# mahilab/mahi-mpc

Hardware: AMD Instinct MI355X
Metric: MPC solves/sec (whole node), nx=4 N=30 batch, at 1/2/4/8 MI355X (higher is better)
Workload: dtype f64; 1 GPU; cfg#2: 2-link arm nx=4 nu=2, N=30, h=2 ms, cold-start SQP (exact or Gauss-Newton Hessian: config.hessian) to ||grad||<=1e-8, ||g||<=1e-10; batch_per_gpu=4096, global_batch=4096, horizon=30, kkt_solver=riccati (16 lanes per instance), hessian=exact (Lagrangian, IPOPT's default), init_states=reference cold start V = 0 (MMPC_INIT_ZERO: V not read)

## Files before the change

### mahi-mpc_amd/csrc/fast_trig.h

```cpp
#pragma once
#include <math.h>

#ifndef MMPC_TRIG_FN
#if defined(__HIPCC__)
#define MMPC_TRIG_FN __device__ __forceinline__
#else
#define MMPC_TRIG_FN inline
#endif
#endif

namespace mmpc {

#define MMPC_TRIG_CONSTANTS                                                                                        \
    {0.63661977236758134308, 1.5707963267948966, 6.123233995736766e-17, -1.4973849048591698e-33,                 \
     -1.66666666666666324348e-01, 8.33333333332248946124e-03, -1.98412698298579493134e-04,                       \
     2.75573137070700676789e-06, -2.50507602534068634195e-08, 1.58969099521155010221e-10,                        \
     4.16666666666666019037e-02, -1.38888888888741095749e-03, 2.48015872894767294178e-05,                        \
     -2.75573143513906633035e-07, 2.08757232129817482790e-09, -1.13596475577881948265e-11}

#if defined(__HIPCC__)
__constant__ double kTrigConst[16] = MMPC_TRIG_CONSTANTS;
using trig_cptr = __attribute__((address_space(4))) const double*;
__device__ __forceinline__ trig_cptr trig_table() {
    trig_cptr K = (trig_cptr)kTrigConst;
    asm volatile("" : "+s"(K));
    return K;
}
#else
static const double kTrigConst[16] = MMPC_TRIG_CONSTANTS;
using trig_cptr = const double*;
inline trig_cptr trig_table() { return kTrigConst; }
#endif
#undef MMPC_TRIG_CONSTANTS

MMPC_TRIG_FN void sincos_fast(trig_cptr K, double x, double* s, double* c) {
#if !defined(__HIPCC__) && !defined(MMPC_TRIG_DEVICE_PATH_ON_HOST)
    if (!(fabs(x) <= 1647099.3291652855)) {
        *s = sin(x);
        *c = cos(x);
        return;
    }
#endif
    const double n = rint(x * K[0]);
    double r = fma(-n, K[1], x);
    r = fma(-n, K[2], r);
    r = fma(-n, K[3], r);
    r = fabs(x) <= 1647099.3291652855 ? r : __builtin_nan("");
    const double z = r * r;
    const double ps = fma(z, fma(z, fma(z, fma(z, K[9], K[8]), K[7]), K[6]), K[5]);
    const double sr = fma(z * r, fma(z, ps, K[4]), r);
    const double pc = z * fma(z, fma(z, fma(z, fma(z, fma(z, K[15], K[14]), K[13]), K[12]), K[11]), K[10]);
    const double hz = 0.5 * z;
    const double w = 1.0 - hz;
    const double cr = w + (((1.0 - w) - hz) + z * pc);
    const int q = (int)fma(-4.0, floor(0.25 * n), n);
    const bool odd = (q & 1) != 0;
    const double a = odd ? cr : sr, b = odd ? sr : cr;
    *s = (q & 2) ? -a : a;
    *c = ((q + 1) & 2) ? -b : b;
}

}
```

### mahi-mpc_amd/csrc/models.h

```cpp
#pragma once
#include <type_traits>

#include "device.h"
#include "exo_model_gen.h"
#include "two_link_fast.h"

namespace mmpc {

struct TwoLinkArm {
    static constexpr int NX = 4;
    static constexpr int NU = 2;
    static constexpr int NQ = 2;
    MMPC_HD static void eval(const double* x, const double* u, double* xd) { TwoLinkFast::eval(x, u, xd); }
    MMPC_HD static void eval_jac(const double* x, const double* u, double* xd, double* fx, double* fu) {
        double Fq[4], Fqd[4], Fu[4];
        TwoLinkFast::eval_acc_jac(x, u, xd + 2, Fq, Fqd, Fu);
        xd[0] = x[2];
        xd[1] = x[3];
#pragma unroll
        for (int r = 0; r < 2; ++r) {
#pragma unroll
            for (int c = 0; c < 4; ++c) fx[r * 4 + c] = (c == 2 + r) ? 1.0 : 0.0;
            fu[r * 2] = fu[r * 2 + 1] = 0.0;
#pragma unroll
            for (int c = 0; c < 2; ++c) {
                fx[(2 + r) * 4 + c] = Fq[r * 2 + c];
                fx[(2 + r) * 4 + 2 + c] = Fqd[r * 2 + c];
                fu[(2 + r) * 2 + c] = Fu[r * 2 + c];
            }
        }
    }
    MMPC_HD static void eval_acc_jac(const double* x, const double* u, double* acc, double* Fq, double* Fqd,
                                     double* Fu) {
        TwoLinkFast::eval_acc_jac(x, u, acc, Fq, Fqd, Fu);
    }
    static constexpr bool kHasHess = true;
    MMPC_HD static void eval_hess(const double* x, const double* u, const double* lam, double* W) {
        TwoLinkFast::eval_hess(x, u, lam, W);
    }
    static constexpr bool kControlAffine = true;
};

template <class M, class = void>
struct HasHess {
    static constexpr bool value = false;
};
template <class M>
struct HasHess<M, std::enable_if_t<M::kHasHess>> {
    static constexpr bool value = true;
};
template <class M, class = void>
struct IsControlAffine {
    static constexpr bool value = false;
};
template <class M>
struct IsControlAffine<M, std::enable_if_t<M::kControlAffine>> {
    static constexpr bool value = true;
};

template <class M, class = void>
struct HasJvp {
    static constexpr bool value = false;
};
template <class M>
struct HasJvp<M, std::enable_if_t<M::kHasJvp>> {
    static constexpr bool value = true;
};
template <class M, class = void>
struct HasJacH {
    static constexpr bool value = false;
};
template <class M>
struct HasJacH<M, std::enable_if_t<M::kHasJacH>> {
    static constexpr bool value = true;
};
template <class M>
MMPC_HD void model_acc_jac_h(const double* x, const double* u, double h, double* acc, double* hFq, double* hFqd,
                             double* hFu) {
    if constexpr (HasJacH<M>::value) M::eval_acc_jac_h(x, u, h, acc, hFq, hFqd, hFu);
}
template <class M>
MMPC_HD void model_jvp(const double* x, const double* u, const double* vx, const double* vu, double* xd, double* jv) {
    if constexpr (HasJvp<M>::value) M::eval_jvp(x, u, vx, vu, xd, jv);
}

struct ExoArm {
    static constexpr int NX = 8;
    static constexpr int NU = 4;
    static constexpr int NQ = 4;

    MMPC_HD static void chol4(const double* a, double* l, double* il) {
        sqrt_rsqrt(a[0], l[0], il[0]);
        l[1] = a[1] * il[0];
        l[3] = a[2] * il[0];
        l[6] = a[3] * il[0];
        sqrt_rsqrt(a[4] - l[1] * l[1], l[2], il[1]);
        l[4] = (a[5] - l[3] * l[1]) * il[1];
        l[7] = (a[6] - l[6] * l[1]) * il[1];
        sqrt_rsqrt(a[7] - l[3] * l[3] - l[4] * l[4], l[5], il[2]);
        l[8] = (a[8] - l[6] * l[3] - l[7] * l[4]) * il[2];
        sqrt_rsqrt(a[9] - l[6] * l[6] - l[7] * l[7] - l[8] * l[8], l[9], il[3]);
    }
    MMPC_HD static void chol4_solve(const double* l, const double* il, const double* b, double* y) {
        const double z0 = b[0] * il[0];
        const double z1 = (b[1] - l[1] * z0) * il[1];
        const double z2 = (b[2] - l[3] * z0 - l[4] * z1) * il[2];
        const double z3 = (b[3] - l[6] * z0 - l[7] * z1 - l[8] * z2) * il[3];
        y[3] = z3 * il[3];
        y[2] = (z2 - l[8] * y[3]) * il[2];
        y[1] = (z1 - l[4] * y[2] - l[7] * y[3]) * il[1];
        y[0] = (z0 - l[1] * y[1] - l[3] * y[2] - l[6] * y[3]) * il[0];
    }

    MMPC_HD static void eval(const double* x, const double* u, double* xd) {
        double s[4], c[4];
        const trig_cptr TK = trig_table();
#pragma unroll
        for (int i = 0; i < 4; ++i) sincos_fast(TK, x[i], &s[i], &c[i]);
        const exo::TrigPowers tp(c[1], c[2], c[3], s[1], s[2], s[3]);
        double Mu[10];
        exo::mass_upper(tp, Mu);
        double l[10], il[4], w[4];
#pragma unroll
        for (int i = 0; i < 4; ++i) w[i] = u[i] - exo::kDamping[i] * x[4 + i] - exo::kGravityGain[i] * s[i];
        chol4(Mu, l, il);
#pragma unroll
        for (int i = 0; i < 4; ++i) xd[i] = x[4 + i];
        chol4_solve(l, il, w, xd + 4);
    }

    template <int J>
    MMPC_HD static void dmass_times(const exo::TrigPowers& tp, const double* v, double* out) {
        double dM[10];
        exo::dmass_upper<J>(tp, dM);
        out[0] = fma(dM[0], v[0], fma(dM[1], v[1], fma(dM[2], v[2], dM[3] * v[3])));
        out[1] = fma(dM[1], v[0], fma(dM[4], v[1], fma(dM[5], v[2], dM[6] * v[3])));
        out[2] = fma(dM[2], v[0], fma(dM[5], v[1], fma(dM[7], v[2], dM[8] * v[3])));
        out[3] = fma(dM[3], v[0], fma(dM[6], v[1], fma(dM[8], v[2], dM[9] * v[3])));
    }

    MMPC_HD static void eval_acc_jac(const double* x, const double* u, double* qdd, double* Fq, double* Fqd,
                                     double* Fu) {
        double s[4], c[4];
        const trig_cptr TK = trig_table();
#pragma unroll
        for (int i = 0; i < 4; ++i) sincos_fast(TK, x[i], &s[i], &c[i]);
        const exo::TrigPowers tp(c[1], c[2], c[3], s[1], s[2], s[3]);
        double Mu[10], l[10], il[4], w[4];
        exo::mass_upper(tp, Mu);
#pragma unroll
        for (int i = 0; i < 4; ++i) w[i] = u[i] - exo::kDamping[i] * x[4 + i] - exo::kGravityGain[i] * s[i];
        chol4(Mu, l, il);
        chol4_solve(l, il, w, qdd);
#pragma unroll
        for (int j = 0; j < 4; ++j) {
            double e[4] = {0.0, 0.0, 0.0, 0.0}, col[4];
            e[j] = 1.0;
            chol4_solve(l, il, e, col);
#pragma unroll
            for (int r = 0; r < 4; ++r) Fu[r * 4 + j] = col[r];
        }
        double rhs[4][4];
#pragma unroll
        for (int r = 0; r < 4; ++r) rhs[0][r] = 0.0;
        dmass_times<1>(tp, qdd, rhs[1]);
        dmass_times<2>(tp, qdd, rhs[2]);
        dmass_times<3>(tp, qdd, rhs[3]);
#pragma unroll
        for (int j = 0; j < 4; ++j) {
#pragma unroll
            for (int r = 0; r < 4; ++r) rhs[j][r] = -rhs[j][r];
            rhs[j][j] -= exo::kGravityGain[j] * c[j];
#pragma unroll
            for (int r = 0; r < 4; ++r) {
                double t = 0.0;
#pragma unroll
                for (int cc = 0; cc < 4; ++cc) t = fma(Fu[r * 4 + cc], rhs[j][cc], t);
                Fq[r * 4 + j] = t;
                Fqd[r * 4 + j] = -Fu[r * 4 + j] * exo::kDamping[j];
            }
        }
    }

    static constexpr bool kHasJvp = true;
    MMPC_HD static void eval_jvp(const double* x, const double* u, const double* vx, const double* vu, double* xd,
                                 double* jv) {
        double s[4], c[4];
        const trig_cptr TK = trig_table();
#pragma unroll
        for (int i = 0; i < 4; ++i) sincos_fast(TK, x[i], &s[i], &c[i]);
        const exo::TrigPowers tp(c[1], c[2], c[3], s[1], s[2], s[3]);
        double Mu[10], l[10], il[4], w[4];
        exo::mass_upper(tp, Mu);
#pragma unroll
        for (int i = 0; i < 4; ++i) w[i] = u[i] - exo::kDamping[i] * x[4 + i] - exo::kGravityGain[i] * s[i];
        chol4(Mu, l, il);
#pragma unroll
        for (int i = 0; i < 4; ++i) xd[i] = x[4 + i];
        double* const qdd = xd + 4;
        chol4_solve(l, il, w, qdd);
        double r[4], t1[4], t2[4], t3[4];
        dmass_times<1>(tp, qdd, t1);
        dmass_times<2>(tp, qdd, t2);
        dmass_times<3>(tp, qdd, t3);
#pragma unroll
        for (int i = 0; i < 4; ++i) {
            double t = fma(-exo::kDamping[i], vx[4 + i], vu[i]);
            t = fma(-exo::kGravityGain[i] * c[i], vx[i], t);
            t = fma(-vx[1], t1[i], t);
            t = fma(-vx[2], t2[i], t);
            r[i] = fma(-vx[3], t3[i], t);
        }
        chol4_solve(l, il, r, jv);
    }

    static constexpr bool kHasJacH = true;
    MMPC_HD static void eval_acc_jac_h(const double* x, const double* u, double h, double* qdd, double* hFq,
                                       double* hFqd, double* hFu) {
        double s[4], c[4];
        const trig_cptr TK = trig_table();
#pragma unroll
        for (int i = 0; i < 4; ++i) sincos_fast(TK, x[i], &s[i], &c[i]);
        const exo::TrigPowers tp(c[1], c[2], c[3], s[1], s[2], s[3]);
        double Mu[10], l[10], il[4], w[4];
        exo::mass_upper(tp, Mu);
#pragma unroll
        for (int i = 0; i < 4; ++i) w[i] = u[i] - exo::kDamping[i] * x[4 + i] - exo::kGravityGain[i] * s[i];
        chol4(Mu, l, il);
        chol4_solve(l, il, w, qdd);
        double Li[4][4];
        Li[0][0] = il[0];
        Li[1][1] = il[1];
        Li[2][2] = il[2];
        Li[3][3] = il[3];
        Li[1][0] = -(l[1] * Li[0][0]) * il[1];
        Li[2][1] = -(l[4] * Li[1][1]) * il[2];
        Li[2][0] = -fma(l[3], Li[0][0], l[4] * Li[1][0]) * il[2];
        Li[3][2] = -(l[8] * Li[2][2]) * il[3];
        Li[3][1] = -fma(l[7], Li[1][1], l[8] * Li[2][1]) * il[3];
        Li[3][0] = -fma(l[6], Li[0][0], fma(l[7], Li[1][0], l[8] * Li[2][0])) * il[3];
        double hLi[4][4], hMi[4][4];
#pragma unroll
        for (int k = 0; k < 4; ++k)
#pragma unroll
            for (int j = 0; j <= k; ++j) hLi[k][j] = h * Li[k][j];
#pragma unroll
        for (int i = 0; i < 4; ++i)
#pragma unroll
            for (int j = i; j < 4; ++j) {
                double t = Li[j][i] * hLi[j][j];
#pragma unroll
                for (int k = j + 1; k < 4; ++k) t = fma(Li[k][i], hLi[k][j], t);
                hMi[i][j] = t;
                hMi[j][i] = t;
            }
        double t1[4], t2[4], t3[4];
        dmass_times<1>(tp, qdd, t1);
        dmass_times<2>(tp, qdd, t2);
        dmass_times<3>(tp, qdd, t3);
        const double* const tj[4] = {nullptr, t1, t2, t3};
#pragma unroll
        for (int r = 0; r < 4; ++r) {
            hFq[r * 4] = hMi[r][0] * (-exo::kGravityGain[0] * c[0]);
#pragma unroll
            for (int j = 1; j < 4; ++j) {
                double t = hMi[r][j] * (-exo::kGravityGain[j] * c[j]);
#pragma unroll
                for (int cc = 0; cc < 4; ++cc) t = fma(-hMi[r][cc], tj[j][cc], t);
                hFq[r * 4 + j] = t;
            }
#pragma unroll
            for (int j = 0; j < 4; ++j) {
                hFu[r * 4 + j] = hMi[r][j];
                hFqd[r * 4 + j] = -hMi[r][j] * exo::kDamping[j];
            }
        }
    }

    static constexpr bool kHasHess = true;
    static constexpr bool kControlAffine = true;
    static constexpr bool kExactDefault = false;
    MMPC_HD static void eval_hess(const double* x, const double* u, const double* lam, double* W) {
        double s[4], c[4];
        const trig_cptr TK = trig_table();
#pragma unroll
        for (int i = 0; i < 4; ++i) sincos_fast(TK, x[i], &s[i], &c[i]);
        const exo::TrigPowers tp(c[1], c[2], c[3], s[1], s[2], s[3]);
        double Mu[10], l[10], il[4], w[4], acc[4], mu[4];
        exo::mass_upper(tp, Mu);
        chol4(Mu, l, il);
#pragma unroll
        for (int i = 0; i < 4; ++i) w[i] = u[i] - exo::kDamping[i] * x[4 + i] - exo::kGravityGain[i] * s[i];
        chol4_solve(l, il, w, acc);
        chol4_solve(l, il, lam, mu);
        double beta[4][4], rho[4][4];
#pragma unroll
        for (int r = 0; r < 4; ++r) beta[0][r] = rho[0][r] = 0.0;
        {
            double nu[4];
            dmass_times<1>(tp, acc, beta[1]);
            dmass_times<1>(tp, mu, nu);
            chol4_solve(l, il, nu, rho[1]);
            dmass_times<2>(tp, acc, beta[2]);
            dmass_times<2>(tp, mu, nu);
            chol4_solve(l, il, nu, rho[2]);
            dmass_times<3>(tp, acc, beta[3]);
            dmass_times<3>(tp, mu, nu);
            chol4_solve(l, il, nu, rho[3]);
        }
        double h2[4][4];
#pragma unroll
        for (int i = 0; i < 4; ++i)
#pragma unroll
            for (int j = 0; j < 4; ++j) h2[i][j] = 0.0;
        d2_bilinear<1, 1>(tp, mu, acc, h2);
        d2_bilinear<1, 2>(tp, mu, acc, h2);
        d2_bilinear<1, 3>(tp, mu, acc, h2);
        d2_bilinear<2, 2>(tp, mu, acc, h2);
        d2_bilinear<2, 3>(tp, mu, acc, h2);
        d2_bilinear<3, 3>(tp, mu, acc, h2);
#pragma unroll
        for (int i = 0; i < 144; ++i) W[i] = 0.0;
#pragma unroll
        for (int i = 0; i < 4; ++i) {
#pragma unroll
            for (int j = i; j < 4; ++j) {
                double t = -h2[i][j];
                if (i == j) t = fma(mu[i] * exo::kGravityGain[i], s[i], t);
#pragma unroll
                for (int r = 0; r < 4; ++r) t = fma(rho[i][r], beta[j][r], fma(rho[j][r], beta[i][r], t));
                t = fma(exo::kGravityGain[j] * c[j], rho[i][j], t);
                t = fma(exo::kGravityGain[i] * c[i], rho[j][i], t);
                W[i * 12 + j] = W[j * 12 + i] = t;
            }
#pragma unroll
            for (int j = 0; j < 4; ++j) {
                W[i * 12 + 4 + j] = W[(4 + j) * 12 + i] = exo::kDamping[j] * rho[i][j];
                W[i * 12 + 8 + j] = W[(8 + j) * 12 + i] = -rho[i][j];
            }
        }
    }
    template <int I, int J>
    MMPC_HD static void d2_bilinear(const exo::TrigPowers& tp, const double* a, const double* b, double (*out)[4]) {
        double d[10], v[4];
        exo::d2mass_upper<I, J>(tp, d);
        v[0] = fma(d[0], b[0], fma(d[1], b[1], fma(d[2], b[2], d[3] * b[3])));
        v[1] = fma(d[1], b[0], fma(d[4], b[1], fma(d[5], b[2], d[6] * b[3])));
        v[2] = fma(d[2], b[0], fma(d[5], b[1], fma(d[7], b[2], d[8] * b[3])));
        v[3] = fma(d[3], b[0], fma(d[6], b[1], fma(d[8], b[2], d[9] * b[3])));
        out[I][J] = out[J][I] = fma(a[0], v[0], fma(a[1], v[1], fma(a[2], v[2], a[3] * v[3])));
    }

    MMPC_HD static void eval_jac(const double* x, const double* u, double* xd, double* fx, double* fu) {
        double qdd[4], Fq[16], Fqd[16], Fu[16];
        eval_acc_jac(x, u, qdd, Fq, Fqd, Fu);
#pragma unroll
        for (int r = 0; r < 4; ++r) {
            xd[r] = x[4 + r];
            xd[4 + r] = qdd[r];
#pragma unroll
            for (int cc = 0; cc < 8; ++cc) fx[r * 8 + cc] = (cc == 4 + r) ? 1.0 : 0.0;
#pragma unroll
            for (int cc = 0; cc < 4; ++cc) {
                fx[(4 + r) * 8 + cc] = Fq[r * 4 + cc];
                fx[(4 + r) * 8 + 4 + cc] = Fqd[r * 4 + cc];
                fu[r * 4 + cc] = 0.0;
                fu[(4 + r) * 4 + cc] = Fu[r * 4 + cc];
            }
        }
    }
};

template <class Model>
MMPC_HD void model_eval_jac(const double* x, const double* u, double* xd, double* fx, double* fu) {
    Model::eval_jac(x, u, xd, fx, fu);
}

template <class Model>
MMPC_HD void model_eval(const double* x, const double* u, double* xd) {
    Model::eval(x, u, xd);
}

}
```

### mahi-mpc_amd/csrc/sqp_group.h

```cpp
#undef MMPC_GROUP_PASS
#if defined(MMPC_GROUP_BODY_ONLY)
#define MMPC_GROUP_PASS 2
#elif !defined(MMPC_SQP_GROUP_H)
#define MMPC_SQP_GROUP_H
#define MMPC_GROUP_PASS 1
#else
#define MMPC_GROUP_PASS 0
#endif
#if MMPC_GROUP_PASS == 1
#include <type_traits>

#include "models.h"
#include "sqp_lane.h"
#include "sqp_wave.h"

namespace mmpc {

template <class Model>
__host__ __device__ constexpr bool w_struct_zero(int, int) { return false; }
template <>
__host__ __device__ constexpr bool w_struct_zero<TwoLinkArm>(int r, int j) { return (r == 0 && j >= 2) || (r >= 2 && (j == 0 || j >= 4)); }
template <class Model>
struct WPack {
    static constexpr int PK = 0, OVER = 0;
    __host__ __device__ static constexpr int col(int) { return 0; }
    __host__ __device__ static constexpr int idx(int, int) { return -1; }
};
template <>
struct WPack<TwoLinkArm> {
    static constexpr int PK = 10, OVER = 3;
    __host__ __device__ static constexpr int col(int i) { return i < 3 ? i : 2 * (i - 1); }
    __host__ __device__ static constexpr int idx(int r, int j) {
        if (w_struct_zero<TwoLinkArm>(r, j)) return -1;
        return col(r) + col(j);
    }
};
template <class Model>
__host__ __device__ constexpr bool wpack_valid() {
    using P = WPack<Model>;
    constexpr int NX = Model::NX, KZ = Model::NX + Model::NU;
    for (int r = 0; r < NX; ++r)
        for (int j = 0; j < KZ; ++j) {
            if (P::idx(r, j) < 0) continue;
            if (P::idx(r, j) >= P::PK || P::idx(r, j) != P::col(r) + P::col(j)) return false;
            for (int r2 = 0; r2 < NX; ++r2)
                for (int j2 = 0; j2 < KZ; ++j2)
                    if (P::idx(r2, j2) == P::idx(r, j) && !((r2 == r && j2 == j) || (r2 == j && j2 == r))) return false;
        }
    return P::OVER == P::col(NX - 1) + P::col(KZ - 1) - (P::PK - 1);
}
static_assert(wpack_valid<TwoLinkArm>(), "W record of the 2-link arm");
template <class Model>
__host__ __device__ constexpr int wpack_col_rep(int j) {
    for (int q = 0; q < j; ++q) {
        bool same = true;
        for (int r = 0; r < Model::NX; ++r) same = same && ((WPack<Model>::idx(r, q) < 0) == (WPack<Model>::idx(r, j) < 0));
        if (same) return q;
    }
    return j;
}
constexpr int kGroupLanes = 16;
constexpr int kGroupsPerWave = 4;

__host__ __device__ constexpr int group_const_doubles(int nx, int nu) {
    return nx + nu < kGroupLanes ? nx + (nx > nu ? nx : nu) : 0;
}
__host__ __device__ constexpr int group_lds_doubles(int nx, int nu, int nq, int N, bool bounded = true,
                                                   bool linear = true, bool xb = false, int kc = 0) {
    return N * (3 * nx + (nx - nq) * (nq + (nx - nq) + nu) + 2 * nu) + 3 * (N + 1) * nx + (bounded ? N * nu : 0) +
           (linear ? (nx - nq) * (nq + (nx - nq) + nu) + nx : 0) +
           (N * ((nx - nq) * nu + nx) >= 2 * (nx - nq) * (nx - nq) ? 0 : 2 * (nx - nq) * (nx - nq)) + kc;
}
template <class Model>
struct GroupLaneOps {
    static constexpr int doubles = 0;
};
template <>
struct GroupLaneOps<TwoLinkArm> {
    static constexpr int doubles = group_const_doubles(TwoLinkArm::NX, TwoLinkArm::NU);
};
__host__ __device__ constexpr int group_hess_doubles(int nx, int nu) { return nx * (nx + nu) + nu * nu; }
__host__ __device__ constexpr int group_ws_doubles(int nx, int nu, int N, bool bounded = true, bool xb = false,
                                                  bool w_onchip = false, bool mehr = false) {
    return N * nu * (nx + nu + 1) + (w_onchip ? 0 : N * group_hess_doubles(nx, nu)) +
           (bounded ? N * nu * (nx + 2 * nu + 1) : 0) + (xb ? 5 * N * (nx + nu) : 0) +
           (mehr ? 2 * N * (nx + nu) + N * ((2 + nu) * kGroupLanes + nu * (nu + 1) / 2 + nu) : 0);
}
static_assert(kGroupsPerWave * group_lds_doubles(4, 2, 2, 30, false, false, false, GroupLaneOps<TwoLinkArm>::doubles) * 8 <= 40960,
              "cfg#2 LDS budget");

struct GroupWork {
    double* ws;
};

template <int O>
__device__ __forceinline__ double row_ror(double v) {
    static_assert(O >= 1 && O < 16, "row rotation");
    return __builtin_amdgcn_update_dpp(v, v, 0x120 + O, 0xf, 0xf, true);
}
__device__ __forceinline__ double group_sum(double v) {
    v += row_ror<8>(v);
    v += row_ror<4>(v);
    v += row_ror<2>(v);
    v += row_ror<1>(v);
    return v;
}
__device__ __forceinline__ double group_min(double v) {
    v = fmin(v, row_ror<8>(v));
    v = fmin(v, row_ror<4>(v));
    v = fmin(v, row_ror<2>(v));
    v = fmin(v, row_ror<1>(v));
    return v;
}
__device__ __forceinline__ double group_max(double v) {
    v = fmax(v, row_ror<8>(v));
    v = fmax(v, row_ror<4>(v));
    v = fmax(v, row_ror<2>(v));
    v = fmax(v, row_ror<1>(v));
    return v;
}
__device__ __forceinline__ double group_bcast(double v, int base) { return __shfl(v, base); }
__device__ __forceinline__ int group_bcast_i(int v, int base) { return __shfl(v, base); }

template <int L>
__device__ __forceinline__ double row_bcast(double v) {
    static_assert(L >= 0 && L < 16, "row lane");
    return __builtin_amdgcn_update_dpp(v, v, 0x150 + L, 0xf, 0xf, true);
}
template <int B, int E, class F>
__device__ __forceinline__ void sfor(F&& f) {
    if constexpr (B < E) {
        f(std::integral_constant<int, B>{});
        sfor<B + 1, E>(static_cast<F&&>(f));
    }
}

template <class Model>
__device__ __forceinline__ void group_model(bool lin, const double* lFq, const double* lFqd, const double* lFu,
                                            const double* lxd, const double* lxs, const double* lus, const double* x,
                                            const double* u, double* xd, double* Fq, double* Fqd, double* Fu,
                                            bool jac) {
    constexpr int NQ = Model::NQ, NU = Model::NU, NA = Model::NX - NQ;
    if (!lin) {
        if (jac) {
            Model::eval_acc_jac(x, u, xd + NQ, Fq, Fqd, Fu);
#pragma unroll
            for (int i = 0; i < NQ; ++i) xd[i] = x[NQ + i];
        } else {
            Model::eval(x, u, xd);
        }
        return;
    }
#pragma unroll
    for (int i = 0; i < NQ; ++i) xd[i] = lxd[i] + (x[NQ + i] - lxs[NQ + i]);
#pragma unroll
    for (int i = 0; i < NA; ++i) {
        double t = lxd[NQ + i];
#pragma unroll
        for (int s = 0; s < (NQ > NA ? NQ : NA); ++s) {
            if (s < NA) t = fma(lFqd[i * NA + s], x[NQ + s] - lxs[NQ + s], t);
            if (s < NQ) t = fma(lFq[i * NQ + s], x[s] - lxs[s], t);
        }
#pragma unroll
        for (int c = 0; c < NU; ++c) t = fma(lFu[i * NU + c], u[c] - lus[c], t);
        xd[NQ + i] = t;
    }
    if (jac) {
#pragma unroll
        for (int i = 0; i < NA * NQ; ++i) Fq[i] = lFq[i];
#pragma unroll
        for (int i = 0; i < NA * NA; ++i) Fqd[i] = lFqd[i];
#pragma unroll
        for (int i = 0; i < NA * NU; ++i) Fu[i] = lFu[i];
    }
}

template <class Model, bool BOUNDED = false, bool XB = false, bool EXACT = false>
__global__ __launch_bounds__(64) void sqp_group_kernel(SolveParams p, GroupWork gw) {
    constexpr bool MEHR = false;
    constexpr bool IB = false;
#endif
#if MMPC_GROUP_PASS != 0
    static_assert(!(BOUNDED && XB), "the interior-point variant handles the control bounds itself");
    static_assert(!MEHR || XB, "the barrier rule belongs to the interior-point variant");
    constexpr int NX = Model::NX, NU = Model::NU, NQ = Model::NQ, NA = NX - NQ, NS = NX + NU, ND = NX + NU;
    constexpr int SQ = NA * NQ > 0 ? NA * NQ : 1;
    constexpr int FQ = NA * NQ, FD = NA * NA, FU = NA * NU;
    static_assert(NQ >= 0 && NA >= NQ, "x = [q; z] with qdot = z[0:NQ]");
    constexpr int G = kGroupLanes;
    extern __shared__ double shm[];
    const int gl = threadIdx.x & (G - 1);
    const int gi = threadIdx.x / G;
    [[maybe_unused]] const int lane0 = threadIdx.x;
    MMPC_PHASE_DECL
    const int gbase = gi * G;
    const int64_t slot = (int64_t)blockIdx.x * p.gpw + gi;
    const bool resume = p.tail_idx != nullptr;
    const bool valid = gi < p.gpw && slot < (resume ? (int64_t)min(*p.tail_count, p.tail_slots) : p.B);
    if (!valid) return;
    const int64_t inst = resume ? (int64_t)p.tail_idx[slot] : slot;
    const int64_t ii = inst;
    const int N = p.N;
    const int NV = NX * (N + 1) + NU * N;
    const double h = p.h;

    constexpr int KC = NX + NU < kGroupLanes ? GroupLaneOps<Model>::doubles : 0;
    double* const sX = shm + gi * group_lds_doubles(NX, NU, NQ, N, BOUNDED, p.is_linear != 0, XB, KC);
    double* const sU = sX + (N + 1) * NX;
    double* const sD = sU + N * NU;
    double* const sDX = sD + (N + 1) * NX;
    double* const sDU = sDX + (N + 1) * NX;
    double* const sF = sDU + N * NU;
    double* const sC = sF + N * NX;
    double* const sFq = sC + N * NX;
    double* const sFqd = sFq + N * FQ;
    double* const sFu = sFqd + N * FD;
    double* const sR = sFu + N * FU;
    double* const sHold = sR + N * NX;
    double* const sLin = sHold + (BOUNDED ? N * NU : 0);
    constexpr int NY = NX + NU;
    constexpr int PK = WPack<Model>::PK;
    constexpr bool WLDS = EXACT && !BOUNDED && !XB && IsControlAffine<Model>::value && PK >= NX && PK <= 2 * NX + NU;
    double* const wK = gw.ws + slot * (int64_t)group_ws_doubles(NX, NU, N, BOUNDED, XB, WLDS, MEHR);
    constexpr int KZ = NX + NU, HW = group_hess_doubles(NX, NU);
    double* const wH = wK + N * NU * (NS + 1);
    double* const sW = sD + NX;
    static_assert(!WLDS || WPack<Model>::OVER <= NX, "the over-read of the last W record stays inside sDU");
    if constexpr (WLDS) {
        if (gl < WPack<Model>::OVER) sW[N * PK + gl] = 0.0;
    }
    constexpr int NR = NS + NU + 1;
    double* const wRel = wH + N * HW;
    bool w_zeros_stored = false;
    double* const sZl = wRel;
    double* const sZu = sZl + N * NY;
    double* const sSg = sZu + N * NY;
    double* const sBb = sSg + N * NY;
    double* const sZg = sBb + N * NY;
    [[maybe_unused]] double* const sCl = sZg + N * NY;
    [[maybe_unused]] double* const sCu = sCl + N * NY;
    constexpr int VL = 2 + NU, VC = NU * (NU + 1) / 2, VS = VC + NU, VR = VL * G + VS;
    [[maybe_unused]] double* const sVr = sCu + N * NY;
    const double* const trg = p.traj + ii * (int64_t)N * NX;

    const double* w = p.weights + ii * p.w_stride;
    double Q[NX], R[NU], Rm[NU], up[NU];
#pragma unroll
    for (int r = 0; r < NX; ++r) Q[r] = w[r];
#pragma unroll
    for (int c = 0; c < NU; ++c) {
        R[c] = w[NX + c];
        Rm[c] = w[NX + NU + c];
        up[c] = p.u_prev[ii * NU + c];
    }
    double lbv[NU], ubv[NU];
    load_bounds<NU, BOUNDED, IB>(p, inst, lbv, ubv);
    constexpr bool DIST = (NS < G);
    static_assert(!MEHR || DIST, "Mehrotra's rule: lane-distributed path");
    constexpr bool CAFF = IsControlAffine<Model>::value;
    static_assert(!EXACT || (DIST && HasHess<Model>::value), "exact Hessian: lane-distributed path, model eval_hess");
    const int r = gl;
    const bool lx = r < NX, lu = r >= NX && r < NS, la = r >= NQ && r < NX;
    const int rx = lx ? r : 0;
    const int ru = lu ? r - NX : 0;
    const int ta = la ? r - NQ : 0;
    const double Qr = lx ? w[rx] : 0.0;
    [[maybe_unused]] const double lqd = r < NQ ? 1.0 : 0.0, lad = la ? 1.0 : 0.0;
    const double lxf = lx ? 1.0 : 0.0;
    int wrow = 0;
#pragma unroll
    for (int r2 = 0; r2 < NX; ++r2)
        if (lx && r == r2) wrow = WPack<Model>::col(r2);
    double wm[KZ];
#pragma unroll
    for (int j = 0; j < KZ; ++j) {
        bool nz = false;
#pragma unroll
        for (int r2 = 0; r2 < NX; ++r2)
            if (lx && r == r2 && WPack<Model>::idx(r2, j) >= 0) nz = true;
        wm[j] = wpack_col_rep<Model>(j) < j ? wm[wpack_col_rep<Model>(j)] : (nz ? 1.0 : 0.0);
    }
    const int rq = r < NQ ? r : 0;
    const double Rr = lu ? w[NX + ru] : 0.0;
    double dgx[NS];
#pragma unroll
    for (int j = 0; j < NS; ++j) dgx[j] = (lx && j == r) ? 1.0 : 0.0;
    double lbr = -INFINITY, ubr = INFINITY;
#pragma unroll
    for (int c = 0; c < NU; ++c)
        if (lu && ru == c) {
            lbr = lbv[c];
            ubr = ubv[c];
        }
    double hq[NQ > 0 ? NQ : 1], hrow[NX], qoh[NX], rdg[NU];
#pragma unroll
    for (int z = 0; z < NQ; ++z) hq[z] = (r == NQ + z) ? h : 0.0;
#pragma unroll
    for (int j = 0; j < NX; ++j) {
        hrow[j] = (r < NQ && j == NQ + r) ? h : 0.0;
        qoh[j] = (j == r) ? Qr : 0.0;
    }
#pragma unroll
    for (int c = 0; c < NU; ++c) rdg[c] = (r == NX + c) ? R[c] : 0.0;
    constexpr bool LOPS = KC > 0;
    double* const sKc = sX + group_lds_doubles(NX, NU, NQ, N, BOUNDED, p.is_linear != 0, XB, KC) - KC;
    using LdsB = const __attribute__((address_space(3))) char*;
    using LdsD = const __attribute__((address_space(3))) double*;
    const LdsB shb = (LdsB)shm;
    auto lds = [](LdsB b) { return *(LdsD)b; };
    auto pin = [](LdsB& b) { asm volatile("" : "+v"(b)); };
    [[maybe_unused]] const LdsB iKc = shb + 8 * (int)(sKc - shm), iKz = iKc + 8 * NX;
    constexpr bool MIRROR = LOPS && NQ > 0 && NQ == NA && (NA - 1) * NA < KC;
    [[maybe_unused]] const double Qa = MIRROR ? w[rx] : Qr;
    [[maybe_unused]] const LdsB iAq =
        la ? shb + 8 * ((int)(sFq - shm) + ta * NQ) : ((r < NQ || MIRROR) ? iKc + 8 * ((NX - 1) - (NQ + rq)) : iKz);
    [[maybe_unused]] const int zAq = la ? 8 * FQ : 0, zAd = la ? 8 * FD : 0, zBr = la ? 8 * FU : 0;
    [[maybe_unused]] const LdsB iAd = la ? shb + 8 * ((int)(sFqd - shm) + ta * NA) : ((r < NQ || MIRROR) ? iAq + 8 * NQ : iKz);
    [[maybe_unused]] const LdsB iBr = la ? shb + 8 * ((int)(sFu - shm) + ta * NU) : iKz;
    constexpr bool ACOLP = LOPS && NQ == NA && (NA - 1) * NA < KC;
    static_assert(!MIRROR || ACOLP, "a mirrored lane reads row 0's column through the per-lane column address");
    [[maybe_unused]] const int zAc = (la || r < NQ) ? 8 * FD : 0;
    [[maybe_unused]] const LdsB iAc = la ? shb + 8 * ((int)(sFqd - shm) + ta) : (r < NQ ? shb + 8 * ((int)(sFq - shm) + rq) : iKc),
                                iAcN = iAc + (N - 1) * zAc;
    if constexpr (LOPS) {
        for (int i = gl; i < KC; i += G) sKc[i] = (i == NX - 1) ? h : 0.0;
    }
    {
        const double* Vin = p.V + ii * (int64_t)NV;
        for (int k = gl; k <= N; k += G) {
#pragma unroll
            for (int r = 0; r < NX; ++r)
                sX[k * NX + r] = (k == 0 || p.init_hold) ? p.x0[ii * NX + r] : (p.init_zero ? 0.0 : Vin[k * ND + r]);
            if (k < N) {
#pragma unroll
                for (int c = 0; c < NU; ++c) {
                    const double v = p.init_zero ? 0.0 : Vin[k * ND + NX + c];
                    sU[k * NU + c] = BOUNDED ? proj(v, lbv[c], ubv[c]) : v;
                }
#pragma unroll
                for (int r = 0; r < NX; ++r) sR[k * NX + r] = trg[k * NX + r];
            }
        }
    }
    const double* const tr = sR;
    double yl[XB ? NY : 1], yu[XB ? NY : 1];
    double mub = (XB && resume) ? p.tail_mub[slot] : kIpMu0;
    if constexpr (XB) {
        load_ip_bounds<NX, NU, IB>(p, inst, yl, yu);
        __builtin_amdgcn_wave_barrier();
        if (resume) {
            const double* const lz = p.tail_lws + (inst >> 6) * p.tail_lws_block + (inst & 63);
            for (int k = gl; k < N; k += G) {
#pragma unroll
                for (int j = 0; j < NY; ++j) {
                    sZl[k * NY + j] = lz[((int64_t)k * p.tail_lws_ss + p.tail_lws_zl + j) * 64];
                    sZu[k * NY + j] = lz[((int64_t)k * p.tail_lws_ss + p.tail_lws_zl + NY + j) * 64];
                }
            }
        } else {
            for (int k = gl; k < N; k += G) {
#pragma unroll
                for (int j = 0; j < NY; ++j) {
                    double& y = j < NX ? sX[(k + 1) * NX + j] : sU[k * NU + j - NX];
                    y = ip_push(y, yl[j], yu[j]);
                    sZl[k * NY + j] = yl[j] > -INFINITY ? 1.0 : 0.0;
                    sZu[k * NY + j] = yu[j] < INFINITY ? 1.0 : 0.0;
                }
            }
        }
    }
    const bool lin = p.is_linear != 0;
    double* const lFq = sLin;
    double* const lFqd = lFq + FQ;
    double* const lFu = lFqd + FD;
    double* const lxd = lFu + FU;
    const double* const lxs = sX;
    if (lin && gl == 0) {
        double acc[NA], x[NX], Fq[SQ], Fqd[FD], Fu[FU];
#pragma unroll
        for (int r = 0; r < NX; ++r) x[r] = p.x0[ii * NX + r];
        Model::eval_acc_jac(x, up, acc, Fq, Fqd, Fu);
#pragma unroll
        for (int i = 0; i < FQ; ++i) lFq[i] = Fq[i];
#pragma unroll
        for (int i = 0; i < FD; ++i) lFqd[i] = Fqd[i];
#pragma unroll
        for (int i = 0; i < FU; ++i) lFu[i] = Fu[i];
#pragma unroll
        for (int i = 0; i < NQ; ++i) lxd[i] = x[NQ + i];
#pragma unroll
        for (int i = 0; i < NA; ++i) lxd[NQ + i] = acc[i];
    }
    __builtin_amdgcn_wave_barrier();
    int status = ST_MAX_ITER;
    int it = 0;
    double kkt = 0.0, mu = resume ? p.tail_mu[slot] : 0.0, pg_prev = (BOUNDED && resume) ? p.tail_mub[slot] : INFINITY;
    bool done = !valid;
    constexpr bool FUSE_FWD = true;
    bool fwd_ready = false;
    double J0n = 0.0, c1n = 0.0, cmaxn = 0.0;
    int nfn = 0;
    MMPC_PHASE(0);
    for (it = resume ? p.tail_it[slot] : 0; !done; ++it) {
        MMPC_PHASE(8);
        __builtin_amdgcn_wave_barrier();
        double J0 = J0n, c1 = c1n, cmax = cmaxn;
        int nonfinite = nfn;
        const bool evalA = !(FUSE_FWD && fwd_ready);
        if (evalA) {
            J0 = 0.0;
            c1 = 0.0;
            cmax = 0.0;
            nonfinite = 0;
            for (int k = gl; k < N; k += G) {
                double x[NX], u[NU], xd[NX], Fq[SQ], Fqd[FD], Fu[FU];
#pragma unroll
                for (int r = 0; r < NX; ++r) x[r] = sX[k * NX + r];
#pragma unroll
                for (int c = 0; c < NU; ++c) u[c] = sU[k * NU + c];
                group_model<Model>(lin, lFq, lFqd, lFu, lxd, lxs, up, x, u, xd, Fq, Fqd, Fu, true);
#pragma unroll
                for (int i = 0; i < FQ; ++i) sFq[k * FQ + i] = h * Fq[i];
#pragma unroll
                for (int i = 0; i < FD; ++i) sFqd[k * FD + i] = h * Fqd[i];
#pragma unroll
                for (int i = 0; i < FU; ++i) sFu[k * FU + i] = h * Fu[i];
#pragma unroll
                for (int r = 0; r < NX; ++r) {
                    const double F = fma(h, xd[r], x[r]);
                    sF[k * NX + r] = F;
                    const double c = F - sX[(k + 1) * NX + r];
                    sC[k * NX + r] = c;
                    cmax = fmax(cmax, fabs(c));
                    c1 += fabs(c);
                    nonfinite |= !isfinite(c);
                    const double e = F - tr[k * NX + r];
                    J0 = fma(e * Q[r], e, J0);
                }
#pragma unroll
                for (int c = 0; c < NU; ++c) {
                    const double um = (k == 0) ? up[c] : sU[(k - 1) * NU + c];
                    const double dif = u[c] - um;
                    J0 = fma(dif * R[c], dif, fma(u[c] * Rm[c], u[c], J0));
                }
            }
        }
        double lsum = 0.0, cmpl0 = 0.0, cmplmu = 0.0;
        if constexpr (XB) {
            for (int k = gl; k < N; k += G) {
#pragma unroll
                for (int j = 0; j < NY; ++j) {
                    const double y = j < NX ? sX[(k + 1) * NX + j] : sU[k * NU + j - NX];
                    double sg, bb, zg;
                    ip_terms(y, yl[j], yu[j], sZl[k * NY + j], sZu[k * NY + j], mub, sg, bb, zg, cmpl0, cmplmu, lsum);
                    sSg[k * NY + j] = sg;
                    if constexpr (MEHR) sBb[k * NY + j] = 0.0;
                    else sBb[k * NY + j] = bb;
                    sZg[k * NY + j] = zg;
                }
            }
            lsum = group_sum(lsum);
            cmpl0 = group_max(cmpl0);
            cmplmu = group_max(cmplmu);
            nonfinite |= !isfinite(lsum);
            __builtin_amdgcn_fence(__ATOMIC_RELEASE, "workgroup");
            __builtin_amdgcn_fence(__ATOMIC_ACQUIRE, "workgroup");
        }
        if (evalA) {
            J0 = group_sum(J0);
            c1 = group_sum(c1);
            cmax = group_max(cmax);
        }
        fwd_ready = false;
        __builtin_amdgcn_wave_barrier();
        MMPC_PHASE(1);

        double gmax = 0.0, lmax = 0.0;
        int fact_ok = 1;
        const double beps = BOUNDED ? fmin(kBoundEps, pg_prev) : 0.0;
        auto backward = [&](int pass) {
            double P[NS][NS], pv[NS], lam[NX], unext[NU];
#define Ps(i, j) ((i) <= (j) ? P[(i)][(j)] : P[(j)][(i)])
#pragma unroll
            for (int a = 0; a < NS; ++a) {
                pv[a] = 0.0;
#pragma unroll
                for (int b = a; b < NS; ++b) P[a][b] = (a == b && a < NX) ? Q[a] : 0.0;
            }
#pragma unroll
            for (int r = 0; r < NX; ++r) {
                const double eb = sX[N * NX + r] - tr[(N - 1) * NX + r];
                pv[r] = Q[r] * eb;
                lam[r] = Q[r] * (sD[N * NX + r] + eb);
                if constexpr (XB) {
                    P[r][r] += sSg[(N - 1) * NY + r];
                    pv[r] += sBb[(N - 1) * NY + r];
                    lam[r] += sZg[(N - 1) * NY + r];
                }
                lmax = fmax(lmax, fabs(lam[r]));
            }
#pragma unroll
            for (int c = 0; c < NU; ++c) unext[c] = 0.0;
            for (int k = N - 1; k >= 0; --k) {
                const double* hFq = sFq + k * FQ;
                const double* hFqd = sFqd + k * FD;
                double hFu[FU], x[NX], u[NU], um[NU], cc[NX], tg[NU];
#pragma unroll
                for (int i = 0; i < FU; ++i) hFu[i] = sFu[k * FU + i];
#pragma unroll
                for (int r = 0; r < NX; ++r) {
                    x[r] = sX[k * NX + r];
                    cc[r] = sC[k * NX + r];
                }
#pragma unroll
                for (int c = 0; c < NU; ++c) {
                    u[c] = sU[k * NU + c];
                    um[c] = (k == 0) ? up[c] : sU[(k - 1) * NU + c];
                }
#pragma unroll
                for (int c = 0; c < NU; ++c) {
                    double g = 0.0;
#pragma unroll
                    for (int s = 0; s < NA; ++s) g = fma(hFu[s * NU + c], lam[NQ + s], g);
                    g = fma(R[c], u[c] - um[c], fma(Rm[c], u[c], g));
                    if (k + 1 < N) g -= R[c] * (unext[c] - u[c]);
                    if (XB) g += sZg[k * NY + NX + c];
                    if (!BOUNDED) {
                        gmax = fmax(gmax, fabs(2.0 * g));
                    } else {
                        gmax = fmax(gmax, fabs(u[c] - proj(u[c] - 2.0 * g, lbv[c], ubv[c])));
                        if (pass == 0) {
                            tg[c] = (u[c] <= lbv[c] + beps && g > 0.0)   ? lbv[c]
                                    : (u[c] >= ubv[c] - beps && g < 0.0) ? ubv[c]
                                                                          : NAN;
                            sHold[k * NU + c] = tg[c];
                        } else {
                            tg[c] = sHold[k * NU + c];
                        }
                    }
                    nonfinite |= !isfinite(g);
                    unext[c] = u[c];
                }
                if (k >= 1) {
                    double ln[NX];
                    at_mul<NQ, NA, double>(h, hFq, hFqd, lam, ln);
#pragma unroll
                    for (int r = 0; r < NX; ++r) {
                        lam[r] = fma(Q[r], sD[k * NX + r] + x[r] - tr[(k - 1) * NX + r], ln[r]);
                        if (XB) lam[r] += sZg[(k - 1) * NY + r];
                        lmax = fmax(lmax, fabs(lam[r]));
                    }
                }
                double Gm[NX][NU];
#pragma unroll
                for (int r = 0; r < NX; ++r)
#pragma unroll
                    for (int c = 0; c < NU; ++c) {
                        double t = Ps(r, NX + c);
#pragma unroll
                        for (int s = 0; s < NA; ++s) t = fma(Ps(r, NQ + s), hFu[s * NU + c], t);
                        Gm[r][c] = t;
                    }
                double mv[NX];
#pragma unroll
                for (int r = 0; r < NX; ++r) {
                    double t = pv[r];
#pragma unroll
                    for (int q = 0; q < NX; ++q) t = fma(Ps(r, q), cc[q], t);
                    mv[r] = t;
                }
                double Hww[NU][NU], Y[NU][NS + 1];
#pragma unroll
                for (int a = 0; a < NU; ++a) {
#pragma unroll
                    for (int b = a; b < NU; ++b) {
                        double t = Ps(NX + a, NX + b);
#pragma unroll
                        for (int s = 0; s < NA; ++s)
                            t = fma(hFu[s * NU + a], Gm[NQ + s][b], fma(Ps(NQ + s, NX + a), hFu[s * NU + b], t));
                        if (a == b) t += R[a] + Rm[a];
                        if (XB && a == b) t += sSg[k * NY + NX + a];
                        Hww[a][b] = t;
                    }
                    double t = fma(R[a], u[a] - um[a], fma(Rm[a], u[a], pv[NX + a]));
                    if (XB) t += sBb[k * NY + NX + a];
#pragma unroll
                    for (int s = 0; s < NA; ++s) t = fma(hFu[s * NU + a], mv[NQ + s], t);
#pragma unroll
                    for (int r = 0; r < NX; ++r) t = fma(Ps(r, NX + a), cc[r], t);
                    Y[a][NS] = t;
                    double ga[NX];
#pragma unroll
                    for (int r = 0; r < NX; ++r) ga[r] = Gm[r][a];
                    at_mul<NQ, NA, double>(h, hFq, hFqd, ga, &Y[a][0]);
#pragma unroll
                    for (int c = 0; c < NU; ++c) Y[a][NX + c] = (a == c) ? -R[a] : 0.0;
                }
                double pex[NS];
                if (BOUNDED) {
                    bool hd[NU], any = false;
                    double dl[NU];
#pragma unroll
                    for (int j = 0; j < NS; ++j) pex[j] = 0.0;
#pragma unroll
                    for (int a = 0; a < NU; ++a) {
                        hd[a] = tg[a] == tg[a];
                        dl[a] = hd[a] ? tg[a] - u[a] : 0.0;
                        any |= hd[a];
                    }
                    if (any) {
#pragma unroll
                        for (int a = 0; a < NU; ++a)
#pragma unroll
                            for (int j = 0; j < NS; ++j) pex[j] = fma(Y[a][j], dl[a], pex[j]);
#pragma unroll
                        for (int b = 0; b < NU; ++b) {
                            double t = Y[b][NS];
#pragma unroll
                            for (int a = 0; a < NU; ++a) t = fma(Hww[a < b ? a : b][a < b ? b : a], dl[a], t);
                            Y[b][NS] = hd[b] ? -dl[b] : t;
                        }
#pragma unroll
                        for (int a = 0; a < NU; ++a) {
#pragma unroll
                            for (int b = a; b < NU; ++b)
                                if (hd[a] || hd[b]) Hww[a][b] = (a == b) ? 1.0 : 0.0;
                            if (hd[a])
#pragma unroll
                                for (int j = 0; j < NS; ++j) Y[a][j] = 0.0;
                        }
                    }
                }
                double Pn[NX][NX], pn[NS];
                if (k >= 1) {
#pragma unroll
                    for (int b = 0; b < NX; ++b) {
                        double row[NX], tcol[NX];
#pragma unroll
                        for (int r = 0; r < NX; ++r) {
                            double t;
                            if (b < NQ) {
                                t = Ps(r, b);
#pragma unroll
                                for (int s = 0; s < NA; ++s) t = fma(hFq[s * NQ + b], Ps(r, NQ + s), t);
                            } else {
                                t = (b - NQ < NQ) ? fma(h, Ps(r, b - NQ), Ps(r, b)) : Ps(r, b);
#pragma unroll
                                for (int s = 0; s < NA; ++s) t = fma(hFqd[s * NA + b - NQ], Ps(r, NQ + s), t);
                            }
                            tcol[r] = t;
                        }
                        at_mul<NQ, NA, double>(h, hFq, hFqd, tcol, row);
#pragma unroll
                        for (int a = 0; a <= b; ++a)
                            Pn[a][b] = row[a] + ((a == b) ? Q[a] + (XB ? sSg[(k - 1) * NY + a] : 0.0) : 0.0);
                    }
                    double t[NX];
                    at_mul<NQ, NA, double>(h, hFq, hFqd, mv, t);
#pragma unroll
                    for (int q = 0; q < NX; ++q) {
                        pn[q] = fma(Q[q], x[q] - tr[(k - 1) * NX + q], t[q]);
                        if (XB) pn[q] += sBb[(k - 1) * NY + q];
                    }
#pragma unroll
                    for (int c = 0; c < NU; ++c) pn[NX + c] = -R[c] * (u[c] - um[c]);
                }
                double Kt[NU][NS + 1];
                if constexpr (NU == 2 && !XB) {
                    const double det = fma(Hww[0][0], Hww[1][1], -Hww[0][1] * Hww[0][1]);
                    fact_ok &= (Hww[0][0] > 0.0) && (det > 0.0) && isfinite(det);
                    const double idet = rcp_nr(det);
                    const double i00 = Hww[1][1] * idet, i11 = Hww[0][0] * idet, i01 = -Hww[0][1] * idet;
#pragma unroll
                    for (int j = 0; j <= NS; ++j) {
                        Kt[0][j] = fma(i00, Y[0][j], i01 * Y[1][j]);
                        Kt[1][j] = fma(i01, Y[0][j], i11 * Y[1][j]);
                    }
                } else {
                    double Ld[NU][NU], il[NU];
#pragma unroll
                    for (int a = 0; a < NU; ++a) {
                        double sd = Hww[a][a];
#pragma unroll
                        for (int q = 0; q < a; ++q) sd = fma(-Ld[a][q], Ld[a][q], sd);
                        fact_ok &= (sd > 0.0) && isfinite(sd);
                        const double sp = fmax(sd, 1e-300);
                        double r = __builtin_amdgcn_rsq(sp);
                        r = r * fma(-0.5 * sp * r, r, 1.5);
                        r = r * fma(-0.5 * sp * r, r, 1.5);
                        Ld[a][a] = sp * r;
                        il[a] = r;
#pragma unroll
                        for (int b = a + 1; b < NU; ++b) {
                            double t = Hww[a][b];
#pragma unroll
                            for (int q = 0; q < a; ++q) t = fma(-Ld[b][q], Ld[a][q], t);
                            Ld[b][a] = t * il[a];
                        }
                    }
#pragma unroll
                    for (int a = 0; a < NU; ++a)
#pragma unroll
                        for (int j = 0; j <= NS; ++j) {
                            double t = Y[a][j];
#pragma unroll
                            for (int q = 0; q < a; ++q) t = fma(-Ld[a][q], Y[q][j], t);
                            Y[a][j] = t * il[a];
                        }
#pragma unroll
                    for (int a = NU - 1; a >= 0; --a)
#pragma unroll
                        for (int j = 0; j <= NS; ++j) {
                            double t = Y[a][j];
#pragma unroll
                            for (int q = a + 1; q < NU; ++q) t = fma(-Ld[q][a], Kt[q][j], t);
                            Kt[a][j] = t * il[a];
                        }
                }
#pragma unroll
                for (int a = 0; a < NU; ++a)
#pragma unroll
                    for (int j = 0; j <= NS; ++j) wK[(k * NU + a) * (NS + 1) + j] = -Kt[a][j];
                if (k == 0) break;
                const double(&YB)[NU][NS + 1] = (NU == 2 && !XB) ? Kt : Y;
#pragma unroll
                for (int a = 0; a < NS; ++a) {
                    double t = pn[a];
#pragma unroll
                    for (int q = 0; q < NU; ++q) t = fma(-Y[q][a], YB[q][NS], t);
                    if (BOUNDED) t += pex[a];
                    pv[a] = t;
#pragma unroll
                    for (int b = a; b < NS; ++b) {
                        double v = (b < NX) ? Pn[a][b] : ((a == b) ? R[a - NX] : 0.0);
#pragma unroll
                        for (int q = 0; q < NU; ++q) v = fma(-Y[q][a], YB[q][b], v);
                        P[a][b] = v;
                    }
                }
            }
#undef Ps
        };
        double dJ = 0.0;
        bool resolve = false;
        auto step_sweep = [&](int pass) {
            dJ = 0.0;
            double dx[NX], dup[NU], um[NU];
#pragma unroll
            for (int r = 0; r < NX; ++r) {
                dx[r] = 0.0;
                sDX[r] = 0.0;
            }
#pragma unroll
            for (int c = 0; c < NU; ++c) {
                dup[c] = 0.0;
                um[c] = up[c];
            }
            constexpr int NK = NU * (NS + 1);
            double nK[NK], nFq[SQ], nFqd[FD], nFu[FU], nF[NX], nc[NX], nr[NX], nu_[NU];
#define GROUP_LOAD_STEP(k_)                                                                        \
        do {                                                                                           \
            const int kk_ = (k_);                                                                      \
            _Pragma("unroll") for (int i_ = 0; i_ < NK; ++i_) nK[i_] = wK[kk_ * NK + i_];              \
            _Pragma("unroll") for (int i_ = 0; i_ < FQ; ++i_) nFq[i_] = sFq[kk_ * FQ + i_];             \
            _Pragma("unroll") for (int i_ = 0; i_ < FD; ++i_) nFqd[i_] = sFqd[kk_ * FD + i_];           \
            _Pragma("unroll") for (int i_ = 0; i_ < FU; ++i_) nFu[i_] = sFu[kk_ * FU + i_];             \
            _Pragma("unroll") for (int r_ = 0; r_ < NX; ++r_) {                                        \
            nF[r_] = sF[kk_ * NX + r_];                                                            \
            nc[r_] = sC[kk_ * NX + r_];                                                            \
            nr[r_] = sR[kk_ * NX + r_];                                                            \
            }                                                                                          \
            _Pragma("unroll") for (int c_ = 0; c_ < NU; ++c_) nu_[c_] = sU[kk_ * NU + c_];             \
        } while (0)
            GROUP_LOAD_STEP(0);
            constexpr int kStepUnroll = NX <= 4 ? 2 : 1;
#pragma unroll kStepUnroll
            for (int k = 0; k < N; ++k) {
                double K[NK], hFq[SQ], hFqd[FD], hFu[FU], Fk[NX], ck[NX], rk[NX], uk[NU];
#pragma unroll
                for (int i = 0; i < NK; ++i) K[i] = nK[i];
#pragma unroll
                for (int i = 0; i < FQ; ++i) hFq[i] = nFq[i];
#pragma unroll
                for (int i = 0; i < FD; ++i) hFqd[i] = nFqd[i];
#pragma unroll
                for (int i = 0; i < FU; ++i) hFu[i] = nFu[i];
#pragma unroll
                for (int r = 0; r < NX; ++r) {
                    Fk[r] = nF[r];
                    ck[r] = nc[r];
                    rk[r] = nr[r];
                }
#pragma unroll
                for (int c = 0; c < NU; ++c) uk[c] = nu_[c];
                if (k + 1 < N) GROUP_LOAD_STEP(k + 1);
                double du[NU];
#pragma unroll
                for (int a = 0; a < NU; ++a) {
                    double t = K[a * (NS + 1) + NS];
#pragma unroll
                    for (int q = 0; q < NX; ++q) t = fma(K[a * (NS + 1) + q], dx[q], t);
#pragma unroll
                    for (int c = 0; c < NU; ++c) t = fma(K[a * (NS + 1) + NX + c], dup[c], t);
                    du[a] = t;
                    sDU[k * NU + a] = t;
                }
                if (BOUNDED && pass + 1 < kBoundPasses) {
#pragma unroll
                    for (int a = 0; a < NU; ++a) {
                        const double hv = sHold[k * NU + a], t = uk[a] + du[a];
                        if (hv != hv && (t < lbv[a] || t > ubv[a])) {
                            sHold[k * NU + a] = t < lbv[a] ? lbv[a] : ubv[a];
                            resolve = true;
                        }
                    }
                }
                double ad[NX];
                a_mul<NQ, NA, double>(h, hFq, hFqd, dx, ad);
#pragma unroll
                for (int s = 0; s < NA; ++s)
#pragma unroll
                    for (int c = 0; c < NU; ++c) ad[NQ + s] = fma(hFu[s * NU + c], du[c], ad[NQ + s]);
#pragma unroll
                for (int r = 0; r < NX; ++r) {
                    const double qe = 2.0 * Q[r] * (Fk[r] - rk[r]);
                    dJ = fma(qe, ad[r], dJ);
                    dx[r] = ad[r] + ck[r];
                    sDX[(k + 1) * NX + r] = dx[r];
                }
#pragma unroll
                for (int c = 0; c < NU; ++c) {
                    const double dif = uk[c] - um[c];
                    dJ = fma(2.0 * R[c] * dif, du[c] - dup[c], fma(2.0 * Rm[c] * uk[c], du[c], dJ));
                    um[c] = uk[c];
                    dup[c] = du[c];
                }
            }
#undef GROUP_LOAD_STEP
        };
        auto colA = [&](double own, const double* acol, const double* vb) {
            double t = lxf * own;
#pragma unroll
            for (int z = 0; z < NQ; ++z) t = fma(hq[z], vb[z], t);
#pragma unroll
            for (int s2 = 0; s2 < NA; ++s2) t = fma(acol[s2], vb[NQ + s2], t);
            return t;
        };
        auto load_arow = [&](int k, double* arow, double* brow) {
#pragma unroll
            for (int s2 = 0; s2 < NQ; ++s2)
                arow[s2] = LOPS ? lds(iAq + __mul24(k, zAq) + 8 * s2) : fma(lad, sFq[k * FQ + ta * NQ + s2], hrow[s2]);
#pragma unroll
            for (int s2 = 0; s2 < NA; ++s2)
                arow[NQ + s2] = LOPS ? lds(iAd + __mul24(k, zAd) + 8 * s2) : fma(lad, sFqd[k * FD + ta * NA + s2], hrow[NQ + s2]);
#pragma unroll
            for (int c = 0; c < NU; ++c) brow[c] = LOPS ? lds(iBr + __mul24(k, zBr) + 8 * c) : lad * sFu[k * FU + ta * NU + c];
        };
        auto d_recursion_dist = [&]() {
            double dr = 0.0;
            if (MIRROR || lx) sD[rx] = 0.0;
            struct Op {
                double q[NQ > 0 ? NQ : 1], d[NA], c;
            };
            LdsB jq = iAq, jd = iAd;
            auto fetch = [&](int k, Op& o) {
#pragma unroll
                for (int s2 = 0; s2 < NQ; ++s2) o.q[s2] = LOPS ? lds(jq + 8 * s2) : sFq[k * FQ + ta * NQ + s2];
#pragma unroll
                for (int s2 = 0; s2 < NA; ++s2) o.d[s2] = LOPS ? lds(jd + 8 * s2) : sFqd[k * FD + ta * NA + s2];
                o.c = sC[k * NX + rx];
                if constexpr (LOPS) {
                    jq += zAq;
                    jd += zAd;
                    pin(jq);
                    pin(jd);
                }
            };
            auto stage = [&](int k, Op& o) {
                double db[NX], arow[NX];
#pragma unroll
                for (int s2 = 0; s2 < NQ; ++s2) arow[s2] = LOPS ? o.q[s2] : fma(lad, o.q[s2], hrow[s2]);
#pragma unroll
                for (int s2 = 0; s2 < NA; ++s2) arow[NQ + s2] = LOPS ? o.d[s2] : fma(lad, o.d[s2], hrow[NQ + s2]);
                const double cr = o.c;
                if constexpr (!MIRROR) fetch(k + 2, o);
                sfor<0, NX>([&](auto I) { db[I] = row_bcast<I>(dr); });
                double t0 = dr + cr, t1 = 0.0;
#pragma unroll
                for (int j = 0; j < NX; ++j) {
                    if (j & 1) t1 = fma(arow[j], db[j], t1);
                    else t0 = fma(arow[j], db[j], t0);
                }
                dr = t0 + t1;
                if (MIRROR || lx) sD[(k + 1) * NX + rx] = dr;
                if constexpr (MIRROR) {
                    __builtin_amdgcn_sched_barrier(0);
                    fetch(k + 2, o);
                }
            };
            Op o0, o1;
            fetch(0, o0);
            fetch(LOPS || N > 1 ? 1 : 0, o1);
            int k = 0;
            for (; k + 1 < N; k += 2) {
                stage(k, o0);
                stage(k + 1, o1);
            }
            if (k < N) stage(k, o0);
        };
        auto load_acol = [&](int k, [[maybe_unused]] LdsB& jc, double* acol) {
            if constexpr (ACOLP) {
#pragma unroll
                for (int t2 = 0; t2 < NA; ++t2) acol[t2] = lds(jc + 8 * t2 * NA);
                jc -= zAc;
                pin(jc);
            } else {
#pragma unroll
                for (int t2 = 0; t2 < NA; ++t2) {
                    double v = lad * sFqd[k * FD + t2 * NA + ta];
                    if constexpr (NQ > 0) v = fma(lqd, sFq[k * FQ + t2 * NQ + rq], v);
                    acol[t2] = v;
                }
            }
        };
        auto adjoint_dist = [&]() {
            double lamr;
            {
                const double eb = (MIRROR || lx) ? sX[N * NX + rx] - tr[(N - 1) * NX + rx] : 0.0;
                lamr = Qa * (sD[N * NX + rx] + eb);
                if constexpr (XB) lamr += (MIRROR ? 1.0 : lxf) * sZg[(N - 1) * NY + rx];
                lmax = fmax(lmax, fabs(lamr));
                if (MIRROR || lx) sD[N * NX + rx] = lamr;
            }
            struct Op {
                double fd[NA], fq[NA], xk, trm, dk, zg;
            };
            [[maybe_unused]] LdsB jc = (!MIRROR || lx) ? iAcN : shb + 8 * ((int)(sFq - shm) + (N - 1) * FD);
            [[maybe_unused]] const int zc = MIRROR ? 8 * FD : zAc;
            auto fetch = [&](int k, Op& o) {
#pragma unroll
                for (int t2 = 0; t2 < NA; ++t2) {
                    if constexpr (ACOLP) {
                        o.fd[t2] = lds(jc + 8 * t2 * NA);
                    } else {
                        o.fd[t2] = sFqd[k * FD + t2 * NA + ta];
                        if constexpr (NQ > 0) o.fq[t2] = sFq[k * FQ + t2 * NQ + rq];
                    }
                }
                if constexpr (ACOLP) {
                    jc -= zc;
                    pin(jc);
                }
                o.xk = sX[k * NX + rx];
                o.trm = tr[(k - 1) * NX + rx];
                o.dk = sD[k * NX + rx];
                if constexpr (XB) o.zg = sZg[(k - 1) * NY + rx];
            };
            auto stage = [&](int k, Op& o, [[maybe_unused]] bool more = true) {
                double acol[NA];
#pragma unroll
                for (int t2 = 0; t2 < NA; ++t2) {
                    if constexpr (ACOLP) {
                        acol[t2] = o.fd[t2];
                    } else {
                        double v = lad * o.fd[t2];
                        if constexpr (NQ > 0) v = fma(lqd, o.fq[t2], v);
                        acol[t2] = v;
                    }
                }
                double qe = Qa * (o.dk + (o.xk - o.trm));
                if constexpr (XB) qe += o.zg;
                if constexpr (!MIRROR) fetch(k >= 3 ? k - 2 : 1, o);
                double lamb[NX];
                sfor<0, NX>([&](auto I) { lamb[I] = row_bcast<I>(lamr); });
                double t0 = lamr + qe, t1 = 0.0;
#pragma unroll
                for (int z = 0; z < NQ; ++z) t1 = fma(hq[z], lamb[z], t1);
#pragma unroll
                for (int s2 = 0; s2 < NA; ++s2) {
                    if (s2 & 1) t1 = fma(acol[s2], lamb[NQ + s2], t1);
                    else t0 = fma(acol[s2], lamb[NQ + s2], t0);
                }
                lamr = t0 + t1;
                lmax = fmax(lmax, fabs(MIRROR ? lamr : lxf * lamr));
                if (MIRROR || lx) sD[k * NX + rx] = lamr;
                if constexpr (MIRROR) {
                    __builtin_amdgcn_sched_barrier(0);
                    if (more) fetch(k - 2, o);
                }
            };
            if (N >= 2) {
                Op o0, o1;
                fetch(N - 1, o0);
                fetch(N >= 3 ? N - 2 : 1, o1);
                int k = N - 1;
                if constexpr (MIRROR) {
                    for (; k >= 4; k -= 2) {
                        stage(k, o0);
                        stage(k - 1, o1);
                    }
                    if (k == 3) {
                        stage(3, o0);
                        stage(2, o1, false);
                        stage(1, o0, false);
                    } else if (k == 2) {
                        stage(2, o0, false);
                        stage(1, o1, false);
                    } else {
                        stage(1, o0, false);
                    }
                } else {
                    for (; k >= 2; k -= 2) {
                        stage(k, o0);
                        stage(k - 1, o1);
                    }
                    if (k == 1) stage(1, o0);
                }
            }
            __builtin_amdgcn_fence(__ATOMIC_RELEASE, "workgroup");
            __builtin_amdgcn_fence(__ATOMIC_ACQUIRE, "workgroup");
            for (int k = gl; k < N; k += G) {
#pragma unroll
                for (int c = 0; c < NU; ++c) {
                    double g = 0.0;
#pragma unroll
                    for (int s2 = 0; s2 < NA; ++s2) g = fma(sFu[k * FU + s2 * NU + c], sD[(k + 1) * NX + NQ + s2], g);
                    const double uk = sU[k * NU + c], um = k == 0 ? up[c] : sU[(k - 1) * NU + c];
                    g = fma(R[c], uk - um, fma(Rm[c], uk, g));
                    if (k < N - 1) g -= R[c] * (sU[(k + 1) * NU + c] - uk);
                    if constexpr (XB) g += sZg[k * NY + NX + c];
                    if constexpr (!BOUNDED) {
                        gmax = fmax(gmax, fabs(2.0 * g));
                    } else {
                        gmax = fmax(gmax, fabs(uk - proj(uk - 2.0 * g, lbv[c], ubv[c])));
                        sHold[k * NU + c] = (uk <= lbv[c] + beps && g > 0.0)   ? lbv[c]
                                            : (uk >= ubv[c] - beps && g < 0.0) ? ubv[c]
                                                                                : NAN;
                    }
                    nonfinite |= !isfinite(g);
                }
            }
        };
        auto backward_dist = [&](bool useW) {
            if constexpr (BOUNDED) {
                __builtin_amdgcn_fence(__ATOMIC_RELEASE, "workgroup");
                __builtin_amdgcn_fence(__ATOMIC_ACQUIRE, "workgroup");
            }
            double Prow[NS], pvr;
            [[maybe_unused]] LdsB jcol = iAcN;
            const double lxm = lx ? 1.0 : 0.0;
            struct Wb {
                double r[KZ], u[NU * NU];
            };
            Wb w0;
            auto load_w = [&](int k, Wb& b) {
#pragma unroll
                for (int j = 0; j < KZ; ++j)
                    b.r[j] = WLDS ? sW[k * PK + wrow + WPack<Model>::col(j)] : wH[k * HW + rx * KZ + j];
                if constexpr (!CAFF) {
#pragma unroll
                    for (int j = 0; j < NU * NU; ++j) b.u[j] = wH[k * HW + NX * KZ + j];
                }
            };
            if (EXACT && useW) {
                load_w(N - 1, w0);
            }
#pragma unroll
            for (int j = 0; j < NS; ++j) Prow[j] = j < NX ? qoh[j] : 0.0;
            pvr = Qr * (lx ? sX[N * NX + rx] - tr[(N - 1) * NX + rx] : 0.0);
            if constexpr (XB) {
                const double sgN = sSg[(N - 1) * NY + rx], bbN = sBb[(N - 1) * NY + rx];
#pragma unroll
                for (int j = 0; j < NX; ++j) Prow[j] = fma(dgx[j], sgN, Prow[j]);
                pvr = fma(lxm, bbN, pvr);
            }
            auto stage = [&](int k, auto last_c, Wb& wb) {
                constexpr bool LAST = decltype(last_c)::value;
#if defined(MMPC_PHASE_TIMING) && defined(MMPC_PHASE_STAGES)
                if (gl == 0 && blockIdx.x < kPhaseWavePhases && k < 32)
                    g_mmpc_phase_cycles[kPhaseStageLog + 128 * blockIdx.x + 32 * gi + k] = __builtin_amdgcn_s_memtime();
#endif
                double hFq[SQ], hFqd[FD], hFu[FU], cc[NX], u[NU], um[NU], acol[NA];
#pragma unroll
                for (int i = 0; i < FQ; ++i) hFq[i] = sFq[k * FQ + i];
#pragma unroll
                for (int i = 0; i < FD; ++i) hFqd[i] = sFqd[k * FD + i];
#pragma unroll
                for (int i = 0; i < FU; ++i) hFu[i] = sFu[k * FU + i];
#pragma unroll
                for (int q = 0; q < NX; ++q) cc[q] = sC[k * NX + q];
#pragma unroll
                for (int c = 0; c < NU; ++c) {
                    u[c] = sU[k * NU + c];
                    um[c] = LAST ? up[c] : sU[(k - 1) * NU + c];
                }
                load_acol(k, jcol, acol);
                double xsgu[XB ? NU : 1], xbbu[XB ? NU : 1], xsgx = 0.0, xbbx = 0.0;
                if constexpr (XB) {
#pragma unroll
                    for (int a = 0; a < NU; ++a) {
                        xsgu[a] = sSg[k * NY + NX + a];
                        xbbu[a] = sBb[k * NY + NX + a];
                    }
                    if constexpr (!LAST) {
                        xsgx = sSg[(k - 1) * NY + rx];
                        xbbx = sBb[(k - 1) * NY + rx];
                    }
                }
                double exr = 0.0, duu = 0.0;
                if constexpr (!LAST) {
                    const double xk = sX[k * NX + rx], trm = tr[(k - 1) * NX + rx];
                    exr = xk - trm;
                    duu = sU[k * NU + ru] - sU[(k - 1) * NU + ru];
                }
                double wr[KZ], wu[NU * NU];
                if constexpr (EXACT) {
#pragma unroll
                    for (int j = 0; j < KZ; ++j) wr[j] = useW ? wb.r[j] : 0.0;
#pragma unroll
                    for (int j = 0; j < NU * NU; ++j) wu[j] = (useW && !CAFF) ? wb.u[j] : 0.0;
                    if (!LAST && useW) load_w(k - 1, wb);
                }
                double T[NU], mv = pvr;
#pragma unroll
                for (int b = 0; b < NU; ++b) {
                    double t = Prow[NX + b];
#pragma unroll
                    for (int s2 = 0; s2 < NA; ++s2) t = fma(Prow[NQ + s2], hFu[s2 * NU + b], t);
                    T[b] = t;
                }
#pragma unroll
                for (int q = 0; q < NX; ++q) mv = fma(Prow[q], cc[q], mv);
                double Tb[NS][NU], mvb[NS];
                sfor<0, NS>([&](auto I) {
#pragma unroll
                    for (int b = 0; b < NU; ++b) Tb[I][b] = row_bcast<I>(T[b]);
                    mvb[I] = row_bcast<I>(mv);
                });
                double Hww[NU][NU], hw[NU];
#pragma unroll
                for (int a = 0; a < NU; ++a) {
#pragma unroll
                    for (int b = a; b < NU; ++b) {
                        double t = Tb[NX + a][b];
#pragma unroll
                        for (int s2 = 0; s2 < NA; ++s2) t = fma(hFu[s2 * NU + a], Tb[NQ + s2][b], t);
                        if (a == b) t += R[a] + Rm[a];
                        if constexpr (EXACT && !CAFF) t += wu[a * NU + b];
                        if constexpr (XB) {
                            if (a == b) t += xsgu[a];
                        }
                        Hww[a][b] = t;
                        Hww[b][a] = t;
                    }
                    double t = fma(R[a], u[a] - um[a], fma(Rm[a], u[a], mvb[NX + a]));
#pragma unroll
                    for (int s2 = 0; s2 < NA; ++s2) t = fma(hFu[s2 * NU + a], mvb[NQ + s2], t);
                    if constexpr (XB) t += xbbu[a];
                    hw[a] = t;
                }
                double Ycol[NU];
#pragma unroll
                for (int a = 0; a < NU; ++a) {
                    double tb[NX];
#pragma unroll
                    for (int q = 0; q < NX; ++q) tb[q] = Tb[q][a];
                    Ycol[a] = colA(T[a], acol, tb) - rdg[a];
                    if constexpr (EXACT) Ycol[a] = fma(WLDS ? wm[NX + a] : lxm, wr[NX + a], Ycol[a]);
                }
                if constexpr (BOUNDED) {
#pragma unroll
                    for (int c0 = 0; c0 < NR; c0 += G) {
                        const int col = c0 + r < NR ? c0 + r : NR - 1;
#pragma unroll
                        for (int a = 0; a < NU; ++a) {
                            double v = hw[a];
#pragma unroll
                            for (int b = 0; b < NU; ++b)
                                if (col == NS + b) v = Hww[a][b];
                            wRel[(k * NU + a) * NR + col] = col < NS ? Ycol[a] : v;
                        }
                    }
                }
                double pexr = 0.0, Rk[NU];
#pragma unroll
                for (int c = 0; c < NU; ++c) Rk[c] = R[c];
                if constexpr (BOUNDED) {
                    bool hd[NU];
                    double dl[NU], hw2[NU];
#pragma unroll
                    for (int a = 0; a < NU; ++a) {
                        const double tg = sHold[k * NU + a];
                        hd[a] = tg == tg;
                        dl[a] = hd[a] ? tg - u[a] : 0.0;
                        pexr = fma(Ycol[a], dl[a], pexr);
                    }
#pragma unroll
                    for (int b = 0; b < NU; ++b) {
                        double t = hw[b];
#pragma unroll
                        for (int a = 0; a < NU; ++a) t = fma(Hww[a][b], dl[a], t);
                        hw2[b] = hd[b] ? -dl[b] : t;
                    }
#pragma unroll
                    for (int a = 0; a < NU; ++a) {
                        hw[a] = hw2[a];
#pragma unroll
                        for (int b = 0; b < NU; ++b)
                            if (hd[a] || hd[b]) Hww[a][b] = (a == b) ? 1.0 : 0.0;
                        if (hd[a]) {
                            Ycol[a] = 0.0;
                            Rk[a] = 0.0;
                        }
                    }
                }
                double Kcol[NU], kff[NU], Ku[NU][NU];
                double Ytil[NU], htil[NU];
                if constexpr (XB) {
                    double Ld[NU][NU], il[NU];
#pragma unroll
                    for (int a = 0; a < NU; ++a) {
                        double sd = Hww[a][a];
#pragma unroll
                        for (int q = 0; q < a; ++q) sd = fma(-Ld[a][q], Ld[a][q], sd);
                        fact_ok &= (sd > 0.0) && isfinite(sd);
                        const double sp = fmax(sd, 1e-300);
                        double rr = __builtin_amdgcn_rsq(sp);
                        rr = rr * fma(-0.5 * sp * rr, rr, 1.5);
                        rr = rr * fma(-0.5 * sp * rr, rr, 1.5);
                        Ld[a][a] = sp * rr;
                        il[a] = rr;
#pragma unroll
                        for (int b = a + 1; b < NU; ++b) {
                            double t = Hww[a][b];
#pragma unroll
                            for (int q = 0; q < a; ++q) t = fma(-Ld[b][q], Ld[a][q], t);
                            Ld[b][a] = t * il[a];
                        }
                    }
#pragma unroll
                    for (int a = 0; a < NU; ++a) {
                        double t = Ycol[a], th = hw[a];
#pragma unroll
                        for (int q = 0; q < a; ++q) {
                            t = fma(-Ld[a][q], Ytil[q], t);
                            th = fma(-Ld[a][q], htil[q], th);
                        }
                        Ytil[a] = t * il[a];
                        htil[a] = th * il[a];
                    }
#pragma unroll
                    for (int a = NU - 1; a >= 0; --a) {
                        double t = Ytil[a], th = htil[a];
#pragma unroll
                        for (int q = a + 1; q < NU; ++q) {
                            t = fma(-Ld[q][a], Kcol[q], t);
                            th = fma(-Ld[q][a], kff[q], th);
                        }
                        Kcol[a] = t * il[a];
                        kff[a] = th * il[a];
                    }
                    if constexpr (MEHR) {
                        double* const rec = sVr + k * VR;
                        double pc = 0.0;
#pragma unroll
                        for (int q = 0; q < NX; ++q) pc = fma(Prow[q], cc[q], pc);
                        rec[r] = pc;
                        rec[G + r] = fma(-Rr, duu, lxm * (Qr * exr));
#pragma unroll
                        for (int a = 0; a < NU; ++a) {
                            rec[(2 + a) * G + r] = Ytil[a];
#pragma unroll
                            for (int q = 0; q < a; ++q) rec[VL * G + a * (a + 1) / 2 + q] = Ld[a][q];
                            rec[VL * G + a * (a + 1) / 2 + a] = il[a];
                            rec[VL * G + VC + a] = fma(R[a], u[a] - um[a], Rm[a] * u[a]);
                        }
                    }
                } else if constexpr (NU == 2) {
                    const double det = fma(Hww[0][0], Hww[1][1], -Hww[0][1] * Hww[0][1]);
                    fact_ok &= (Hww[0][0] > 0.0) && (det > 0.0) && isfinite(det);
                    const double idet = rcp_nr(det);
                    const double i00 = Hww[1][1] * idet, i11 = Hww[0][0] * idet, i01 = -Hww[0][1] * idet;
                    Kcol[0] = fma(i00, Ycol[0], i01 * Ycol[1]);
                    Kcol[1] = fma(i01, Ycol[0], i11 * Ycol[1]);
                    kff[0] = fma(i00, hw[0], i01 * hw[1]);
                    kff[1] = fma(i01, hw[0], i11 * hw[1]);
                    Ku[0][0] = -i00 * Rk[0];
                    Ku[0][1] = -i01 * Rk[1];
                    Ku[1][0] = -i01 * Rk[0];
                    Ku[1][1] = -i11 * Rk[1];
                } else {
                    double Ld[NU][NU], il[NU];
#pragma unroll
                    for (int a = 0; a < NU; ++a) {
                        double sd = Hww[a][a];
#pragma unroll
                        for (int q = 0; q < a; ++q) sd = fma(-Ld[a][q], Ld[a][q], sd);
                        fact_ok &= (sd > 0.0) && isfinite(sd);
                        const double sp = fmax(sd, 1e-300);
                        double rr = __builtin_amdgcn_rsq(sp);
                        rr = rr * fma(-0.5 * sp * rr, rr, 1.5);
                        rr = rr * fma(-0.5 * sp * rr, rr, 1.5);
                        Ld[a][a] = sp * rr;
                        il[a] = rr;
#pragma unroll
                        for (int b = a + 1; b < NU; ++b) {
                            double t = Hww[a][b];
#pragma unroll
                            for (int q = 0; q < a; ++q) t = fma(-Ld[b][q], Ld[a][q], t);
                            Ld[b][a] = t * il[a];
                        }
                    }
                    auto chol_solve = [&](const double* rhs, double* out) {
                        double y[NU];
#pragma unroll
                        for (int a = 0; a < NU; ++a) {
                            double t = rhs[a];
#pragma unroll
                            for (int q = 0; q < a; ++q) t = fma(-Ld[a][q], y[q], t);
                            y[a] = t * il[a];
                        }
#pragma unroll
                        for (int a = NU - 1; a >= 0; --a) {
                            double t = y[a];
#pragma unroll
                            for (int q = a + 1; q < NU; ++q) t = fma(-Ld[q][a], out[q], t);
                            out[a] = t * il[a];
                        }
                    };
                    chol_solve(Ycol, Kcol);
                    chol_solve(hw, kff);
#pragma unroll
                    for (int c = 0; c < NU; ++c) {
                        double e[NU], o[NU];
#pragma unroll
                        for (int a = 0; a < NU; ++a) e[a] = (a == c) ? -Rk[c] : 0.0;
                        chol_solve(e, o);
#pragma unroll
                        for (int a = 0; a < NU; ++a) Ku[a][c] = o[a];
                    }
                }
                {
                    const int col = r < NS ? r : NS;
#pragma unroll
                    for (int a = 0; a < NU; ++a) wK[(k * NU + a) * (NS + 1) + col] = -(r < NS ? Kcol[a] : kff[a]);
                }
                if constexpr (LAST) return;
                double Pb[NX][NX];
                sfor<0, NX>([&](auto I) {
#pragma unroll
                    for (int j = I; j < NX; ++j) {
                        Pb[I][j] = row_bcast<I>(Prow[j]);
                        Pb[j][I] = Pb[I][j];
                    }
                });
                double Ur[NX], Pn[NX];
#pragma unroll
                for (int j = 0; j < NX; ++j) {
                    double pc[NX];
#pragma unroll
                    for (int q = 0; q < NX; ++q) pc[q] = Pb[q][j];
                    Ur[j] = colA(Prow[j], acol, pc);
                }
                at_mul<NQ, NA, double>(h, hFq, hFqd, Ur, Pn);
                double pn = fma(-Rr, duu, lxm * fma(Qr, exr, colA(mv, acol, mvb)));
                double sgk = 0.0;
                if constexpr (XB) {
                    sgk = xsgx;
                    pn = fma(lxm, xbbx, pn);
                }
                if constexpr (XB) {
                    double Yb[NU][NS];
                    sfor<0, NS>([&](auto I) {
#pragma unroll
                        for (int a = 0; a < NU; ++a) Yb[a][I] = row_bcast<I>(Ytil[a]);
                    });
#pragma unroll
                    for (int j = 0; j < NS; ++j) {
                        double v = j < NX ? fma(dgx[j], sgk, Pn[j] + qoh[j]) : rdg[j - NX];
                        if constexpr (EXACT) {
                            if (j < NX) v = fma(lxm, wr[j], v);
                        }
#pragma unroll
                        for (int a = 0; a < NU; ++a) v = fma(-Ytil[a], Yb[a][j], v);
                        Prow[j] = v;
                    }
                    double pv2 = pn;
#pragma unroll
                    for (int a = 0; a < NU; ++a) pv2 = fma(-Ytil[a], htil[a], pv2);
                    pvr = pv2;
                    return;
                }
                double Kb[NU][NX];
                sfor<0, NX>([&](auto I) {
#pragma unroll
                    for (int a = 0; a < NU; ++a) Kb[a][I] = row_bcast<I>(Kcol[a]);
                });
#pragma unroll
                for (int j = 0; j < NS; ++j) {
                    double v = j < NX ? Pn[j] + qoh[j] : rdg[j - NX];
                    if constexpr (EXACT) {
                        if (j < NX) v = fma(WLDS ? wm[j] : lxm, wr[j], v);
                    }
#pragma unroll
                    for (int a = 0; a < NU; ++a) v = fma(-Ycol[a], j < NX ? Kb[a][j] : Ku[a][j - NX], v);
                    Prow[j] = v;
                }
                double pv2 = pn;
#pragma unroll
                for (int a = 0; a < NU; ++a) pv2 = fma(-Ycol[a], kff[a], pv2);
                if constexpr (BOUNDED) pv2 += pexr;
                pvr = pv2;
            };
            using F_ = std::false_type;
            if constexpr (BOUNDED || (XB && EXACT)) {
                for (int k = N - 1; k >= 1; --k) stage(k, F_{}, w0);
                stage(0, std::true_type{}, w0);
            } else if ((N - 1) & 1) {
                stage(N - 1, F_{}, w0);
                for (int k = N - 2; k >= 2; k -= 2) {
                    stage(k, F_{}, w0);
                    stage(k - 1, F_{}, w0);
                }
                stage(0, std::true_type{}, w0);
            } else {
                for (int k = N - 1; k >= 2; k -= 2) {
                    stage(k, F_{}, w0);
                    stage(k - 1, F_{}, w0);
                }
                stage(0, std::true_type{}, w0);
            }
        };
        [[maybe_unused]] auto backward_vec = [&]() {
            if constexpr (MEHR) {
                const double lxm = lx ? 1.0 : 0.0;
                [[maybe_unused]] LdsB jcol = iAcN;
                double pvr = Qr * (lx ? sX[N * NX + rx] - tr[(N - 1) * NX + rx] : 0.0);
                pvr = fma(lxm, sBb[(N - 1) * NY + rx], pvr);
                struct Rec {
                    double pc, pn0, yt[NU], sh[VS], bbu[NU], bbx;
                };
                auto fetch = [&](int k, Rec& o) {
                    const double* const rec = sVr + k * VR;
                    o.pc = rec[r];
                    o.pn0 = rec[G + r];
#pragma unroll
                    for (int a = 0; a < NU; ++a) {
                        o.yt[a] = rec[(2 + a) * G + r];
                        o.bbu[a] = sBb[k * NY + NX + a];
                    }
#pragma unroll
                    for (int i = 0; i < VS; ++i) o.sh[i] = rec[VL * G + i];
                    o.bbx = sBb[(k > 0 ? k - 1 : 0) * NY + rx];
                };
                auto stage = [&](int k, const Rec& o) {
                    double hFu[FU], acol[NA];
#pragma unroll
                    for (int i = 0; i < FU; ++i) hFu[i] = sFu[k * FU + i];
                    load_acol(k, jcol, acol);
                    const double mv = pvr + o.pc;
                    double mvb[NS];
                    sfor<0, NS>([&](auto I) { mvb[I] = row_bcast<I>(mv); });
                    double htil[NU], kff[NU];
#pragma unroll
                    for (int a = 0; a < NU; ++a) {
                        double t = o.sh[VC + a] + mvb[NX + a];
#pragma unroll
                        for (int s2 = 0; s2 < NA; ++s2) t = fma(hFu[s2 * NU + a], mvb[NQ + s2], t);
                        t += o.bbu[a];
#pragma unroll
                        for (int q = 0; q < a; ++q) t = fma(-o.sh[a * (a + 1) / 2 + q], htil[q], t);
                        htil[a] = t * o.sh[a * (a + 1) / 2 + a];
                    }
#pragma unroll
                    for (int a = NU - 1; a >= 0; --a) {
                        double t = htil[a];
#pragma unroll
                        for (int q = a + 1; q < NU; ++q) t = fma(-o.sh[q * (q + 1) / 2 + a], kff[q], t);
                        kff[a] = t * o.sh[a * (a + 1) / 2 + a];
                    }
#pragma unroll
                    for (int a = 0; a < NU; ++a) wK[(k * NU + a) * (NS + 1) + NS] = -kff[a];
                    if (k == 0) return;
                    double pv2 = fma(lxm, colA(mv, acol, mvb) + o.bbx, o.pn0);
#pragma unroll
                    for (int a = 0; a < NU; ++a) pv2 = fma(-o.yt[a], htil[a], pv2);
                    pvr = pv2;
                };
                Rec o0, o1;
                fetch(N - 1, o0);
                int k = N - 1;
                for (; k >= 1; k -= 2) {
                    fetch(k - 1, o1);
                    stage(k, o0);
                    fetch(k >= 2 ? k - 2 : 0, o0);
                    stage(k - 1, o1);
                }
                if (k == 0) stage(0, o0);
            }
        };
        if constexpr (DIST) {
            d_recursion_dist();
            adjoint_dist();
            lmax = group_max(lmax);
            gmax = group_max(gmax);
        } else if (gl == 0) {
            {
                double d[NX];
#pragma unroll
                for (int r = 0; r < NX; ++r) {
                    d[r] = 0.0;
                    sD[r] = 0.0;
                }
                double aq[SQ], ad[FD], ac[NX];
#pragma unroll
                for (int i = 0; i < FQ; ++i) aq[i] = sFq[i];
#pragma unroll
                for (int i = 0; i < FD; ++i) ad[i] = sFqd[i];
#pragma unroll
                for (int r = 0; r < NX; ++r) ac[r] = sC[r];
                constexpr int kDUnroll = NX <= 4 ? 2 : 1;
#pragma unroll kDUnroll
                for (int k = 0; k < N; ++k) {
                    double fq[SQ], fd[FD], cc[NX], dn[NX];
#pragma unroll
                    for (int i = 0; i < FQ; ++i) fq[i] = aq[i];
#pragma unroll
                    for (int i = 0; i < FD; ++i) fd[i] = ad[i];
#pragma unroll
                    for (int r = 0; r < NX; ++r) cc[r] = ac[r];
                    const int kn = k + 1 < N ? k + 1 : k;
#pragma unroll
                    for (int i = 0; i < FQ; ++i) aq[i] = sFq[kn * FQ + i];
#pragma unroll
                    for (int i = 0; i < FD; ++i) ad[i] = sFqd[kn * FD + i];
#pragma unroll
                    for (int r = 0; r < NX; ++r) ac[r] = sC[kn * NX + r];
                    a_mul<NQ, NA, double>(h, fq, fd, d, dn);
#pragma unroll
                    for (int r = 0; r < NX; ++r) {
                        d[r] = dn[r] + cc[r];
                        sD[(k + 1) * NX + r] = d[r];
                    }
                }
            }
            backward(0);
        }
        if constexpr (!DIST) {
            gmax = group_bcast(gmax, gbase);
            lmax = group_bcast(lmax, gbase);
            fact_ok = group_bcast_i(fact_ok, gbase);
        }
        MMPC_PHASE(2);
        nonfinite = (group_max((double)nonfinite) != 0.0);
        kkt = fmax(gmax, cmax);
        if (XB) kkt = fmax(kkt, 2.0 * cmpl0);
        double* trc = p.trace && valid ? p.trace + (inst * (p.max_iter + 1) + it) * 8 : nullptr;
        if (trc && gl == 0) {
            trc[0] = gmax;
            trc[1] = cmax;
            trc[2] = J0;
            trc[3] = c1;
            trc[7] = lmax;
        }
        if (nonfinite || !isfinite(kkt)) {
            status = ST_NONFINITE;
            break;
        }
        if (gmax <= p.tol_grad && cmax <= p.tol_defect && (!XB || 2.0 * cmpl0 <= kIpTolCompl)) {
            status = ST_CONVERGED;
            break;
        }
        if (it == p.max_iter) {
            status = ST_MAX_ITER;
            break;
        }
        MMPC_PHASE(9);
        if constexpr (EXACT) {
            __builtin_amdgcn_wave_barrier();
            auto w_stage = [&](int k) {
                double x[NX], u[NU], la[NA], W[KZ * KZ];
#pragma unroll
                for (int r2 = 0; r2 < NX; ++r2) x[r2] = sX[k * NX + r2];
#pragma unroll
                for (int c = 0; c < NU; ++c) u[c] = sU[k * NU + c];
#pragma unroll
                for (int s2 = 0; s2 < NA; ++s2) la[s2] = h * sD[(k + 1) * NX + NQ + s2];
                if constexpr (WLDS) __builtin_amdgcn_wave_barrier();
                Model::eval_hess(x, u, la, W);
                if constexpr (WLDS) {
                    static_assert(!WLDS || PK >= NX, "write order of the W pass");
#pragma unroll
                    for (int r2 = 0; r2 < NX; ++r2)
#pragma unroll
                        for (int j = r2; j < KZ; ++j)
                            if (WPack<Model>::idx(r2, j) >= 0) sW[k * PK + WPack<Model>::idx(r2, j)] = W[r2 * KZ + j];
                } else {
                    double* const dst = wH + k * HW;
#pragma unroll
                    for (int r2 = 0; r2 < NX; ++r2)
#pragma unroll
                        for (int j = 0; j < KZ; ++j)
                            if (!w_struct_zero<Model>(r2, j) || !w_zeros_stored) dst[r2 * KZ + j] = W[r2 * KZ + j];
                    if constexpr (!CAFF) {
#pragma unroll
                        for (int a = 0; a < NU; ++a)
#pragma unroll
                            for (int b = 0; b < NU; ++b) dst[NX * KZ + a * NU + b] = W[(NX + a) * KZ + NX + b];
                    }
                }
            };
            if constexpr (WLDS) {
                for (int k0 = ((N - 1) / G) * G; k0 >= 0; k0 -= G)
                    if (k0 + gl < N) w_stage(k0 + gl);
                MMPC_PHASE(9);
                __builtin_amdgcn_wave_barrier();
            } else {
                for (int k = gl; k < N; k += G) w_stage(k);
                w_zeros_stored = true;
                MMPC_PHASE(9);
                __builtin_amdgcn_fence(__ATOMIC_RELEASE, "workgroup");
                __builtin_amdgcn_fence(__ATOMIC_ACQUIRE, "workgroup");
            }
        }
        bool use_w = EXACT;
        if constexpr (DIST) {
            backward_dist(use_w);
            if (EXACT && !fact_ok) {
                fact_ok = 1;
                use_w = false;
                backward_dist(false);
            }
        }
        if (!fact_ok) {
            status = ST_FACT_FAILED;
            break;
        }
        if (BOUNDED) pg_prev = gmax;
        const double mub_next = (XB && fmax(fmax(0.5 * gmax, cmax), cmplmu) <= kIpKappaEps * mub)
                                    ? fmax(kIpTolCompl / 20.0, fmin(kIpKappaMu * mub, pow(mub, kIpThetaMu)))
                                    : mub;

        MMPC_PHASE(3);
        if constexpr (DIST) {
            auto step_dist = [&](bool check) {
                __builtin_amdgcn_fence(__ATOMIC_RELEASE, "workgroup");
                __builtin_amdgcn_fence(__ATOMIC_ACQUIRE, "workgroup");
                constexpr bool RUN = MIRROR;
                double sr = 0.0;
                if (RUN || lx) sDX[rx] = 0.0;
                constexpr int NK = NS + 1;
                const double* const Kp = wK + ru * NK;
                struct Ops {
                    double K[NK], a[NX], b[NU], c, Rw[BOUNDED ? NR : 1];
                };
                const double* const Rp = wRel + ru * NR;
                using LdsW = __attribute__((address_space(3))) double*;
                [[maybe_unused]] LdsB ja = iAq, jd = iAd, jb = iBr, jcs = shb + 8 * ((int)(sC - shm) + rx);
                [[maybe_unused]] LdsB js = shb + 8 * (lu ? (int)(sDU - shm) + ru : (int)(sDX - shm) + NX + rx);
                [[maybe_unused]] LdsB jt = shb + 8 * (lu ? (int)(sD - shm) + ru : (int)(sD - shm) + NX + rx);
                [[maybe_unused]] const int zs = lu ? 8 * NU : 8 * NX, zt = lu ? 0 : 8 * NX;
                using GlbD = const __attribute__((address_space(1))) double*;
                [[maybe_unused]] GlbD jK = (GlbD)Kp;
                [[maybe_unused]] GlbD jR = (GlbD)Rp;
                [[maybe_unused]] auto refill = [&](Ops& o) {
#pragma unroll
                    for (int j = 0; j < NK; ++j) o.K[j] = jK[j];
#pragma unroll
                    for (int s2 = 0; s2 < NQ; ++s2) o.a[s2] = lds(ja + 8 * s2);
#pragma unroll
                    for (int s2 = 0; s2 < NA; ++s2) o.a[NQ + s2] = lds(jd + 8 * s2);
#pragma unroll
                    for (int c = 0; c < NU; ++c) o.b[c] = lds(jb + 8 * c);
                    o.c = lds(jcs);
                    if constexpr (BOUNDED) {
#pragma unroll
                        for (int j = 0; j < NR; ++j) o.Rw[j] = jR[j];
                    }
                };
                [[maybe_unused]] auto advance = [&]() {
                    ja += zAq;
                    jd += zAd;
                    jb += zBr;
                    jcs += 8 * NX;
                    jK += NU * NK;
                    pin(ja);
                    pin(jd);
                    pin(jb);
                    pin(jcs);
                    asm volatile("" : "+v"(jK));
                    if constexpr (BOUNDED) {
                        jR += NU * NR;
                        asm volatile("" : "+v"(jR));
                    }
                };
                auto fetch = [&](int k, Ops& o) {
#pragma unroll
                    for (int j = 0; j < NK; ++j) o.K[j] = Kp[k * NU * NK + j];
                    load_arow(k, o.a, o.b);
                    o.c = sC[k * NX + rx];
                    if constexpr (BOUNDED) {
#pragma unroll
                        for (int j = 0; j < NR; ++j) o.Rw[j] = Rp[k * NU * NR + j];
                    }
                };
                auto stage = [&](int k, Ops& o, [[maybe_unused]] bool more = true) {
                    double sb[NS];
                    sfor<0, NS>([&](auto I) { sb[I] = row_bcast<I>(sr); });
                    double du0 = o.K[NS], du1 = 0.0;
#pragma unroll
                    for (int j = 0; j < NS; ++j) {
                        if (j & 1) du1 = fma(o.K[j], sb[j], du1);
                        else du0 = fma(o.K[j], sb[j], du0);
                    }
                    const double du = du0 + du1;
                    double ad = sr;
#pragma unroll
                    for (int j = 0; j < NX; ++j) ad = fma(o.a[j], sb[j], ad);
                    double dub[NU];
                    sfor<0, NU>([&](auto I) { dub[I] = row_bcast<NX + I>(du); });
#pragma unroll
                    for (int c = 0; c < NU; ++c) ad = fma(o.b[c], dub[c], ad);
                    const double dxn = ad + o.c;
                    if constexpr (RUN) {
                        sr = lu ? du : dxn;
                        *(LdsW)js = sr;
                        *(LdsW)jt = ad;
                        js += zs;
                        jt += zt;
                        pin(js);
                        pin(jt);
                    } else {
                        if (lx) {
                            sDX[(k + 1) * NX + rx] = dxn;
                            sD[(k + 1) * NX + rx] = ad;
                        }
                        if (lu) sDU[k * NU + ru] = du;
                    }
                    if constexpr (BOUNDED) {
                        if (check && lu) {
                            const double hv = sHold[k * NU + ru], t = sU[k * NU + ru] + du;
                            if (hv != hv) {
                                if (t < lbr || t > ubr) {
                                    sHold[k * NU + ru] = t < lbr ? lbr : ubr;
                                    resolve = true;
                                }
                            } else if (!p.no_release) {
                                double m = o.Rw[NR - 1];
#pragma unroll
                                for (int j = 0; j < NS; ++j) m = fma(o.Rw[j], sb[j], m);
#pragma unroll
                                for (int b = 0; b < NU; ++b) m = fma(o.Rw[NS + b], dub[b], m);
                                if ((hv == lbr && m < 0.0) || (hv == ubr && m > 0.0)) {
                                    sHold[k * NU + ru] = NAN;
                                    resolve = true;
                                }
                            }
                        }
                    }
                    if constexpr (RUN) {
                        if (more) {
                            refill(o);
                            advance();
                        }
                    } else {
                        sr = lx ? dxn : (lu ? du : 0.0);
                        fetch(k + 3 < N ? k + 3 : N - 1, o);
                    }
                };
                Ops o0, o1, o2;
                if constexpr (RUN) {
                    refill(o0);
                    if (N > 1) advance();
                    refill(o1);
                    if (N > 2) advance();
                    refill(o2);
                    advance();
                    int k = 0;
                    for (; k + 5 < N; k += 3) {
                        stage(k, o0, true);
                        stage(k + 1, o1, true);
                        stage(k + 2, o2, true);
                    }
                    const int left = N - 3 - k;
                    if (left == 1) {
                        stage(k, o0, true);
                        stage(k + 1, o1, false);
                        stage(k + 2, o2, false);
                        stage(k + 3, o0, false);
                    } else if (left == 2) {
                        stage(k, o0, true);
                        stage(k + 1, o1, true);
                        stage(k + 2, o2, false);
                        stage(k + 3, o0, false);
                        stage(k + 4, o1, false);
                    } else {
                        stage(k, o0, false);
                        if (N >= 2) stage(k + 1, o1, false);
                        if (N >= 3) stage(k + 2, o2, false);
                    }
                    return;
                }
                fetch(0, o0);
                fetch(N > 1 ? 1 : 0, o1);
                fetch(N > 2 ? 2 : 0, o2);
                if (N % 3 == 1) {
                    stage(0, o0);
                    for (int k = 1; k < N; k += 3) {
                        stage(k, o1);
                        stage(k + 1, o2);
                        stage(k + 2, o0);
                    }
                } else if (N % 3 == 2) {
                    stage(0, o0);
                    stage(1, o1);
                    for (int k = 2; k < N; k += 3) {
                        stage(k, o2);
                        stage(k + 1, o0);
                        stage(k + 2, o1);
                    }
                } else {
                    for (int k = 0; k < N; k += 3) {
                        stage(k, o0);
                        stage(k + 1, o1);
                        stage(k + 2, o2);
                    }
                }
            };
            if constexpr (MEHR) {
                step_dist(false);
                __builtin_amdgcn_wave_barrier();
                double ap = 1.0, ad = 1.0, sz = 0.0;
                for (int k = gl; k < N; k += G) {
#pragma unroll
                    for (int j = 0; j < NY; ++j) {
                        const double y = j < NX ? sX[(k + 1) * NX + j] : sU[k * NU + j - NX];
                        const double dy = j < NX ? sDX[(k + 1) * NX + j] : sDU[k * NU + j - NX];
                        ip_aff_limits(y, dy, yl[j], yu[j], sZl[k * NY + j], sZu[k * NY + j], ap, ad, sz);
                    }
                }
                ap = group_min(ap);
                ad = group_min(ad);
                sz = group_sum(sz);
                double saff = 0.0;
                for (int k = gl; k < N; k += G) {
#pragma unroll
                    for (int j = 0; j < NY; ++j) {
                        const double y = j < NX ? sX[(k + 1) * NX + j] : sU[k * NU + j - NX];
                        const double dy = j < NX ? sDX[(k + 1) * NX + j] : sDU[k * NU + j - NX];
                        saff += ip_aff_compl(y, dy, yl[j], yu[j], sZl[k * NY + j], sZu[k * NY + j], ap, ad);
                    }
                }
                saff = group_sum(saff);
                int nb = 0;
#pragma unroll
                for (int j = 0; j < NY; ++j) nb += (yl[j] > -INFINITY) + (yu[j] < INFINITY);
                const double mbnd = (double)nb * (double)N;
                const double muc = sz / mbnd, mua = saff / mbnd;
                const double sig = muc > 0.0 ? pow(mua / muc, 3.0) : 0.0;
                mub = fmax(kIpTolCompl / 20.0, fmin(sig * muc, kIpMu0));
                for (int k = gl; k < N; k += G) {
#pragma unroll
                    for (int j = 0; j < NY; ++j) {
                        const double y = j < NX ? sX[(k + 1) * NX + j] : sU[k * NU + j - NX];
                        const double dy = j < NX ? sDX[(k + 1) * NX + j] : sDU[k * NU + j - NX];
                        double ccl, ccu, bb;
                        ip_corrector(y, dy, yl[j], yu[j], sZl[k * NY + j], sZu[k * NY + j], mub, ccl, ccu, bb);
                        sCl[k * NY + j] = ccl;
                        sCu[k * NY + j] = ccu;
                        sBb[k * NY + j] = bb;
                    }
                }
                __builtin_amdgcn_fence(__ATOMIC_RELEASE, "workgroup");
                __builtin_amdgcn_fence(__ATOMIC_ACQUIRE, "workgroup");
                backward_vec();
            }
            for (int pass = 0;; ++pass) {
                if (pass > 0) {
                    __builtin_amdgcn_fence(__ATOMIC_RELEASE, "workgroup");
                    __builtin_amdgcn_fence(__ATOMIC_ACQUIRE, "workgroup");
                    backward_dist(use_w);
                    if (EXACT && use_w && !fact_ok) {
                        fact_ok = 1;
                        use_w = false;
                        backward_dist(false);
                    }
                    if (!fact_ok) break;
                }
                resolve = false;
                const int passes = (it == 0 && !p.no_release) ? 2 : kBoundPasses;
                step_dist(BOUNDED && pass + 1 < passes);
                if constexpr (!BOUNDED) {
                    break;
                } else {
                    resolve = group_max(resolve ? 1.0 : 0.0) != 0.0;
                    if (!resolve || pass + 1 >= passes) break;
                }
            }
            __builtin_amdgcn_wave_barrier();
            double dj = 0.0;
            for (int k = gl; k < N; k += G) {
#pragma unroll
                for (int q = 0; q < NX; ++q) dj = fma(2.0 * Q[q] * (sF[k * NX + q] - tr[k * NX + q]), sD[(k + 1) * NX + q], dj);
#pragma unroll
                for (int c = 0; c < NU; ++c) {
                    const double uk = sU[k * NU + c], duk = sDU[k * NU + c];
                    const double um = (k == 0) ? up[c] : sU[(k - 1) * NU + c];
                    const double dum = (k == 0) ? 0.0 : sDU[(k - 1) * NU + c];
                    dj = fma(2.0 * R[c] * (uk - um), duk - dum, fma(2.0 * Rm[c] * uk, duk, dj));
                }
            }
            dJ = group_sum(dj);
        } else {
            if (gl == 0) {
                for (int pass = 0;; ++pass) {
                    if (pass > 0) backward(pass);
                    if (!fact_ok) break;
                    resolve = false;
                    step_sweep(pass);
                    if (!BOUNDED || !resolve || pass + 1 >= kBoundPasses) break;
                }
            }
            fact_ok = group_bcast_i(fact_ok, gbase);
            dJ = group_bcast(dJ, gbase);
        }
        if (!fact_ok) {
            status = ST_FACT_FAILED;
            break;
        }
        __builtin_amdgcn_wave_barrier();
        MMPC_PHASE(4);
        double amax = 1.0, az = 1.0, dbar = 0.0;
        if constexpr (XB) {
            const double tau = kIpTau;
            for (int k = gl; k < N; k += G) {
#pragma unroll
                for (int j = 0; j < NY; ++j) {
                    const double y = j < NX ? sX[(k + 1) * NX + j] : sU[k * NU + j - NX];
                    const double dy = j < NX ? sDX[(k + 1) * NX + j] : sDU[k * NU + j - NX];
                    if constexpr (MEHR)
                        ip_step_limits_pc(y, dy, yl[j], yu[j], sZl[k * NY + j], sZu[k * NY + j], mub, tau,
                                          sCl[k * NY + j], sCu[k * NY + j], amax, az, dbar);
                    else
                        ip_step_limits(y, dy, yl[j], yu[j], sZl[k * NY + j], sZu[k * NY + j], mub, tau, sBb[k * NY + j],
                                       amax, az, dbar);
                }
            }
            amax = group_min(amax);
            az = group_min(az);
            dbar = group_sum(dbar);
        }

        mu = fmax(mu, 4.0 * lmax + 1.0);
        const double phi0 = XB ? fma(mu, c1, fma(-2.0 * mub, lsum, J0)) : fma(mu, c1, J0);
        const double dphi = XB ? dJ + dbar - mu * c1 : dJ - mu * c1;
        double alpha = amax;
        bool accepted = false;
        double ctm = 0.0;
        int nft = 0;
        auto trial = [&](auto jac_c, double& Jt, double& ct, double& lt) {
            constexpr bool JAC = decltype(jac_c)::value;
            for (int k = gl; k < N; k += G) {
                double x[NX], u[NU], xd[NX];
#pragma unroll
                for (int r = 0; r < NX; ++r) x[r] = fma(alpha, sDX[k * NX + r], sX[k * NX + r]);
#pragma unroll
                for (int c = 0; c < NU; ++c) {
                    u[c] = fma(alpha, sDU[k * NU + c], sU[k * NU + c]);
                    if (BOUNDED) u[c] = proj(u[c], lbv[c], ubv[c]);
                }
                if constexpr (JAC) {
                    double Fq[SQ], Fqd[FD], Fu[FU];
                    group_model<Model>(lin, lFq, lFqd, lFu, lxd, lxs, up, x, u, xd, Fq, Fqd, Fu, true);
#pragma unroll
                    for (int i = 0; i < FQ; ++i) sFq[k * FQ + i] = h * Fq[i];
#pragma unroll
                    for (int i = 0; i < FD; ++i) sFqd[k * FD + i] = h * Fqd[i];
#pragma unroll
                    for (int i = 0; i < FU; ++i) sFu[k * FU + i] = h * Fu[i];
#pragma unroll
                    for (int r = 0; r < NX; ++r) {
                        const double F = fma(h, xd[r], x[r]);
                        sF[k * NX + r] = F;
                        const double c = F - fma(alpha, sDX[(k + 1) * NX + r], sX[(k + 1) * NX + r]);
                        sC[k * NX + r] = c;
                        ctm = fmax(ctm, fabs(c));
                        ct += fabs(c);
                        nft |= !isfinite(c);
                        const double er = F - tr[k * NX + r];
                        Jt = fma(er * Q[r], er, Jt);
                    }
                } else {
                    group_model<Model>(lin, lFq, lFqd, lFu, lxd, lxs, up, x, u, xd, nullptr, nullptr, nullptr, false);
#pragma unroll
                    for (int r = 0; r < NX; ++r) {
                        const double F = fma(h, xd[r], x[r]);
                        const double er = F - tr[k * NX + r];
                        Jt = fma(er * Q[r], er, Jt);
                        ct += fabs(F - fma(alpha, sDX[(k + 1) * NX + r], sX[(k + 1) * NX + r]));
                    }
                }
#pragma unroll
                for (int c = 0; c < NU; ++c) {
                    double um = (k == 0) ? up[c] : fma(alpha, sDU[(k - 1) * NU + c], sU[(k - 1) * NU + c]);
                    if (BOUNDED && k > 0) um = proj(um, lbv[c], ubv[c]);
                    const double dif = u[c] - um;
                    Jt = fma(dif * R[c], dif, fma(u[c] * Rm[c], u[c], Jt));
                }
                if constexpr (XB) {
#pragma unroll
                    for (int j = 0; j < NY; ++j) {
                        const double y = j < NX ? fma(alpha, sDX[(k + 1) * NX + j], sX[(k + 1) * NX + j]) : u[j - NX];
                        lt += ip_log_slacks(y, yl[j], yu[j]);
                    }
                }
            }
        };
        bool jac_trial = false;
        for (int ls = 0; ls < 30; ++ls) {
            double Jt = 0.0, ct = 0.0, lt = 0.0;
            jac_trial = FUSE_FWD && ls == 0;
            if (jac_trial) trial(std::true_type{}, Jt, ct, lt);
            else trial(std::false_type{}, Jt, ct, lt);
            Jt = group_sum(Jt);
            ct = group_sum(ct);
            if (XB) lt = group_sum(lt);
            const double phit = XB ? fma(mu, ct, fma(-2.0 * mub, lt, Jt)) : fma(mu, ct, Jt);
            const double noise = 1.0 + fabs(phi0);
            if (dphi >= -1e-11 * noise || phit <= phi0 + 1e-4 * alpha * dphi + 1e-13 * noise ||
                (!XB && it == 0 && first_iter_filter_accepts(J0, c1, Jt, ct, dJ, alpha))) {
                accepted = true;
                if (FUSE_FWD && jac_trial) {
                    fwd_ready = true;
                    J0n = Jt;
                    c1n = ct;
                    cmaxn = group_max(ctm);
                    nfn = nft;
                }
                break;
            }
            alpha *= 0.5;
        }
        if (trc && gl == 0) {
            trc[4] = XB ? amax : dJ;
            trc[5] = alpha;
            trc[6] = XB ? mub : mu;
            if (XB) trc[3] = cmpl0;
        }
        MMPC_PHASE(5);
        if (!accepted) {
            status = ST_LS_FAILED;
            break;
        }
        __builtin_amdgcn_wave_barrier();
        if constexpr (XB) {
            for (int k = gl; k < N; k += G) {
#pragma unroll
                for (int j = 0; j < NY; ++j) {
                    double& y = j < NX ? sX[(k + 1) * NX + j] : sU[k * NU + j - NX];
                    const double dy = j < NX ? sDX[(k + 1) * NX + j] : sDU[k * NU + j - NX];
                    double zl = sZl[k * NY + j], zu = sZu[k * NY + j], yn;
                    if constexpr (MEHR)
                        ip_update_pc(y, dy, yl[j], yu[j], zl, zu, mub, sCl[k * NY + j], sCu[k * NY + j], alpha, az, yn);
                    else
                        ip_update(y, dy, yl[j], yu[j], zl, zu, mub, alpha, az, yn);
                    y = yn;
                    sZl[k * NY + j] = zl;
                    sZu[k * NY + j] = zu;
                }
            }
            if constexpr (!MEHR) mub = mub_next;
        } else {
            for (int k = gl; k <= N; k += G) {
                if (k > 0) {
#pragma unroll
                    for (int r = 0; r < NX; ++r) sX[k * NX + r] = fma(alpha, sDX[k * NX + r], sX[k * NX + r]);
                }
                if (k < N) {
#pragma unroll
                    for (int c = 0; c < NU; ++c) {
                        const double un = fma(alpha, sDU[k * NU + c], sU[k * NU + c]);
                        sU[k * NU + c] = BOUNDED ? proj(un, lbv[c], ubv[c]) : un;
                    }
                }
            }
        }
    }
    __builtin_amdgcn_wave_barrier();
    MMPC_PHASE(6);
    if (!valid) return;
    double* Vout = p.V + inst * (int64_t)NV;
    for (int k = gl; k <= N; k += G) {
#pragma unroll
        for (int r = 0; r < NX; ++r) Vout[k * ND + r] = sX[k * NX + r];
        if (k < N) {
#pragma unroll
            for (int c = 0; c < NU; ++c) Vout[k * ND + NX + c] = sU[k * NU + c];
        }
    }
    if (p.u0_out && gl < NU) p.u0_out[inst * NU + gl] = sU[gl];
    if (gl == 0) {
        if (p.status) p.status[inst] = status;
        if (p.iters) p.iters[inst] = it;
        if (p.kkt) p.kkt[inst] = kkt;
    }
    MMPC_PHASE(7);
    MMPC_PHASE_FLUSH
#endif
#if MMPC_GROUP_PASS == 1
}

template <class Model, bool EXACT = false>
__global__ __launch_bounds__(64) void sqp_group_mehrotra_kernel(SolveParams p, GroupWork gw) {
    constexpr bool BOUNDED = false, XB = true, MEHR = true;
    constexpr bool IB = false;
#define MMPC_GROUP_BODY_ONLY
#include "sqp_group.h"
#undef MMPC_GROUP_BODY_ONLY
}

template <class Model, bool BOUNDED, bool XB, bool EXACT = false, bool MEHR = false>
__global__ __launch_bounds__(64) void sqp_group_instb_kernel(SolveParams p, GroupWork gw) {
    static_assert(BOUNDED || XB, "per-instance bounds: the bounded variants only");
    constexpr bool IB = true;
#define MMPC_GROUP_BODY_ONLY
#include "sqp_group.h"
#undef MMPC_GROUP_BODY_ONLY
}

}
#endif
```

### mahi-mpc_amd/csrc/two_link_fast.h

```cpp
#pragma once
#include "fast_trig.h"

namespace mmpc {

struct TwoLinkFast {
    static constexpr double kG = 9.81;
    struct Terms {
        double sA, cA, sB, cB, sAB, cAB, E, F, iD, nA, nB;
    };
    MMPC_HD static void terms(const double* x, const double* u, Terms& t) {
        const trig_cptr TK = trig_table();
        sincos_fast(TK, x[0], &t.sA, &t.cA);
        sincos_fast(TK, x[1], &t.sB, &t.cB);
        t.cAB = fma(t.cA, t.cB, -t.sA * t.sB);
        t.sAB = fma(t.sA, t.cB, t.cA * t.sB);
        t.E = 1.0 + t.cB;
        t.F = fma(2.0, t.cB, 3.0);
        t.iD = 1.0 / fma(t.cB, t.cB, -2.0);
        const double dA = x[2], dB = x[3], TA = u[0], TB = u[1], dS = dA + dB;
        t.nA = fma(-t.E, TB, TA) + t.sB * fma(dS, dS, t.cB * dA * dA) + kG * fma(t.cB, t.cAB, -2.0 * t.cA);
        t.nB = fma(t.E, TA, -t.F * TB) + t.sB * fma(t.F * dA, dA, t.E * dB * fma(2.0, dA, dB)) +
               kG * fma(2.0 + t.cB, t.cAB, -2.0 * t.E * t.cA);
    }
    MMPC_HD static void eval(const double* x, const double* u, double* xd) {
        Terms t;
        terms(x, u, t);
        xd[0] = x[2];
        xd[1] = x[3];
        xd[2] = -t.nA * t.iD;
        xd[3] = t.nB * t.iD;
    }
    MMPC_HD static void grads(const double* x, const double* u, const Terms& t, double* gA, double* gB) {
        const double dA = x[2], dB = x[3], TA = u[0], TB = u[1], dS = dA + dB;
        const double c2s2 = fma(t.cB, t.cB, -t.sB * t.sB);
        gA[0] = kG * fma(-t.cB, t.sAB, 2.0 * t.sA);
        gA[1] = t.sB * TB + t.cB * dS * dS + c2s2 * dA * dA - kG * fma(t.sB, t.cAB, t.cB * t.sAB);
        gA[2] = 2.0 * t.sB * fma(t.cB, dA, dS);
        gA[3] = 2.0 * t.sB * dS;
        gA[4] = 1.0;
        gA[5] = -t.E;
        const double Q = fma(t.F * dA, dA, t.E * dB * fma(2.0, dA, dB));
        const double P = dA * fma(2.0, dA, 2.0 * dB) + dB * dB;
        gB[0] = kG * fma(-(2.0 + t.cB), t.sAB, 2.0 * t.E * t.sA);
        gB[1] = fma(-t.sB, TA, 2.0 * t.sB * TB) + fma(t.cB, Q, -t.sB * t.sB * P) +
                kG * (fma(-t.sB, t.cAB, -(2.0 + t.cB) * t.sAB) + 2.0 * t.sB * t.cA);
        gB[2] = 2.0 * t.sB * fma(t.F, dA, t.E * dB);
        gB[3] = 2.0 * t.E * t.sB * dS;
        gB[4] = t.E;
        gB[5] = -t.F;
    }
    MMPC_HD static void eval_acc_jac(const double* x, const double* u, double* acc, double* Fq, double* Fqd, double* Fu) {
        Terms t;
        terms(x, u, t);
        double gA[6], gB[6];
        grads(x, u, t, gA, gB);
        const double aA = -t.nA * t.iD, aB = t.nB * t.iD;
        acc[0] = aA;
        acc[1] = aB;
        const double rD = -2.0 * t.cB * t.sB * t.iD;
        Fq[0] = -gA[0] * t.iD;
        Fq[1] = fma(-gA[1], t.iD, -aA * rD);
        Fq[2] = gB[0] * t.iD;
        Fq[3] = fma(gB[1], t.iD, -aB * rD);
        Fqd[0] = -gA[2] * t.iD;
        Fqd[1] = -gA[3] * t.iD;
        Fqd[2] = gB[2] * t.iD;
        Fqd[3] = gB[3] * t.iD;
        Fu[0] = -gA[4] * t.iD;
        Fu[1] = -gA[5] * t.iD;
        Fu[2] = gB[4] * t.iD;
        Fu[3] = gB[5] * t.iD;
    }
    MMPC_HD static void eval_hess(const double* x, const double* u, const double* lam, double* W) {
        Terms t;
        terms(x, u, t);
        double gA[6], gB[6];
        grads(x, u, t, gA, gB);
        const double dA = x[2], dB = x[3], TA = u[0], TB = u[1], dS = dA + dB;
        const double l0 = -lam[0], l1 = lam[1];
        const double c2s2 = fma(t.cB, t.cB, -t.sB * t.sB);
        const double Q = fma(t.F * dA, dA, t.E * dB * fma(2.0, dA, dB));
        const double P = dA * fma(2.0, dA, 2.0 * dB) + dB * dB;
        const double A00 = kG * fma(-t.cB, t.cAB, 2.0 * t.cA);
        const double A01 = kG * fma(t.sB, t.sAB, -t.cB * t.cAB);
        const double A11 = t.cB * TB - t.sB * dS * dS - 4.0 * t.cB * t.sB * dA * dA -
                           2.0 * kG * fma(t.cB, t.cAB, -t.sB * t.sAB);
        const double A12 = 2.0 * fma(t.cB, dS, c2s2 * dA), A13 = 2.0 * t.cB * dS, A15 = t.sB;
        const double A22 = 2.0 * t.sB * t.E, A23 = 2.0 * t.sB, A33 = 2.0 * t.sB;
        const double B00 = kG * fma(-(2.0 + t.cB), t.cAB, 2.0 * t.E * t.cA);
        const double B01 = kG * (fma(t.sB, t.sAB, -(2.0 + t.cB) * t.cAB) - 2.0 * t.sB * t.sA);
        const double B11 = fma(-t.cB, TA, 2.0 * t.cB * TB) - t.sB * fma(3.0 * t.cB, P, Q) +
                           2.0 * kG * (fma(-t.E, t.cAB, t.sB * t.sAB) + t.cB * t.cA);
        const double B12 = fma(t.cB, 2.0 * fma(t.F, dA, t.E * dB), -t.sB * t.sB * (4.0 * dA + 2.0 * dB));
        const double B13 = 2.0 * dS * fma(t.E, t.cB, -t.sB * t.sB), B14 = -t.sB, B15 = 2.0 * t.sB;
        const double B22 = 2.0 * t.F * t.sB, B23 = 2.0 * t.E * t.sB, B33 = 2.0 * t.E * t.sB;
        double H[6][6];
#pragma unroll
        for (int i = 0; i < 6; ++i)
#pragma unroll
            for (int j = 0; j < 6; ++j) H[i][j] = 0.0;
        H[0][0] = fma(l0, A00, l1 * B00);
        H[0][1] = fma(l0, A01, l1 * B01);
        H[1][1] = fma(l0, A11, l1 * B11);
        H[1][2] = fma(l0, A12, l1 * B12);
        H[1][3] = fma(l0, A13, l1 * B13);
        H[1][4] = l1 * B14;
        H[1][5] = fma(l0, A15, l1 * B15);
        H[2][2] = fma(l0, A22, l1 * B22);
        H[2][3] = fma(l0, A23, l1 * B23);
        H[3][3] = fma(l0, A33, l1 * B33);
        double gp[6];
#pragma unroll
        for (int j = 0; j < 6; ++j) gp[j] = fma(l0, gA[j], l1 * gB[j]);
        const double psi = fma(l0, t.nA, l1 * t.nB);
        const double Dp = -2.0 * t.cB * t.sB, Dpp = -2.0 * c2s2;
        const double iD = t.iD, iD2 = iD * iD;
#pragma unroll
        for (int i = 0; i < 6; ++i)
#pragma unroll
            for (int j = i; j < 6; ++j) {
                double v = H[i][j] * iD;
                if (j == 1) v = fma(-gp[i] * Dp, iD2, v);
                if (i == 1) v = fma(-gp[j] * Dp, iD2, v);
                if (i == 1 && j == 1) v = fma(psi, fma(2.0 * Dp * Dp, iD, -Dpp) * iD2, v);
                W[i * 6 + j] = v;
                W[j * 6 + i] = v;
            }
    }
};

}
```

Baseline: 30.60 million solves/s.

## Evaluate model dynamics, Jacobians and Hessians for two stages per lane with packed types

Adds a dpack<W> value type and templates the two-link model's terms, gradients, Jacobian and Hessian on it. Each lane now evaluates two horizon stages together, with interleaved sincos polynomials, in the linearization and exact-Hessian passes, and the prologue initialization is restructured to match. The aim is more instruction-level parallelism in the long dependent FMA chains of the f64 model evaluation. In exchange, register pressure rises, and odd stage counts need duplicate-stage masking.

New measurement: 31.31 million solves/s, median of 6. +2.3%, better.

```diff
diff --git a/mahi-mpc_amd/csrc/fast_trig.h b/mahi-mpc_amd/csrc/fast_trig.h
--- a/mahi-mpc_amd/csrc/fast_trig.h
+++ b/mahi-mpc_amd/csrc/fast_trig.h
@@ -60,4 +60,43 @@
     *c = ((q + 1) & 2) ? -b : b;
 }
 
+template <int W>
+MMPC_TRIG_FN void sincos_fast_w(trig_cptr K, const double* x, double* s, double* c) {
+#if !defined(__HIPCC__) && !defined(MMPC_TRIG_DEVICE_PATH_ON_HOST)
+    for (int e = 0; e < W; ++e) sincos_fast(K, x[e], s + e, c + e);
+#else
+#define MMPC_W for (int e = 0; e < W; ++e)
+    double n[W], r[W], z[W], ps[W], pc[W], sr[W], cr[W];
+    MMPC_W n[e] = rint(x[e] * K[0]);
+    MMPC_W r[e] = fma(-n[e], K[1], x[e]);
+    MMPC_W r[e] = fma(-n[e], K[2], r[e]);
+    MMPC_W r[e] = fma(-n[e], K[3], r[e]);
+    MMPC_W r[e] = fabs(x[e]) <= 1647099.3291652855 ? r[e] : __builtin_nan("");
+    MMPC_W z[e] = r[e] * r[e];
+    MMPC_W ps[e] = fma(z[e], K[9], K[8]);
+    MMPC_W pc[e] = fma(z[e], K[15], K[14]);
+    MMPC_W ps[e] = fma(z[e], ps[e], K[7]);
+    MMPC_W pc[e] = fma(z[e], pc[e], K[13]);
+    MMPC_W ps[e] = fma(z[e], ps[e], K[6]);
+    MMPC_W pc[e] = fma(z[e], pc[e], K[12]);
+    MMPC_W ps[e] = fma(z[e], ps[e], K[5]);
+    MMPC_W pc[e] = fma(z[e], pc[e], K[11]);
+    MMPC_W sr[e] = fma(z[e] * r[e], fma(z[e], ps[e], K[4]), r[e]);
+    MMPC_W pc[e] = z[e] * fma(z[e], pc[e], K[10]);
+    MMPC_W {
+        const double hz = 0.5 * z[e];
+        const double w = 1.0 - hz;
+        cr[e] = w + (((1.0 - w) - hz) + z[e] * pc[e]);
+    }
+    MMPC_W {
+        const int q = (int)fma(-4.0, floor(0.25 * n[e]), n[e]);
+        const bool odd = (q & 1) != 0;
+        const double a = odd ? cr[e] : sr[e], b = odd ? sr[e] : cr[e];
+        s[e] = (q & 2) ? -a : a;
+        c[e] = ((q + 1) & 2) ? -b : b;
+    }
+#undef MMPC_W
+#endif
 }
+
+}
diff --git a/mahi-mpc_amd/csrc/models.h b/mahi-mpc_amd/csrc/models.h
--- a/mahi-mpc_amd/csrc/models.h
+++ b/mahi-mpc_amd/csrc/models.h
@@ -11,7 +11,9 @@
     static constexpr int NX = 4;
     static constexpr int NU = 2;
     static constexpr int NQ = 2;
-    MMPC_HD static void eval(const double* x, const double* u, double* xd) { TwoLinkFast::eval(x, u, xd); }
+    static constexpr bool kWideEval = true;
+    template <class T>
+    MMPC_HD static void eval(const T* x, const T* u, T* xd) { TwoLinkFast::eval(x, u, xd); }
     MMPC_HD static void eval_jac(const double* x, const double* u, double* xd, double* fx, double* fu) {
         double Fq[4], Fqd[4], Fu[4];
         TwoLinkFast::eval_acc_jac(x, u, xd + 2, Fq, Fqd, Fu);
@@ -30,12 +32,13 @@
             }
         }
     }
-    MMPC_HD static void eval_acc_jac(const double* x, const double* u, double* acc, double* Fq, double* Fqd,
-                                     double* Fu) {
+    template <class T>
+    MMPC_HD static void eval_acc_jac(const T* x, const T* u, T* acc, T* Fq, T* Fqd, T* Fu) {
         TwoLinkFast::eval_acc_jac(x, u, acc, Fq, Fqd, Fu);
     }
     static constexpr bool kHasHess = true;
-    MMPC_HD static void eval_hess(const double* x, const double* u, const double* lam, double* W) {
+    template <class T>
+    MMPC_HD static void eval_hess(const T* x, const T* u, const T* lam, T* W) {
         TwoLinkFast::eval_hess(x, u, lam, W);
     }
     static constexpr bool kControlAffine = true;
@@ -47,6 +50,14 @@
 };
 template <class M>
 struct HasHess<M, std::enable_if_t<M::kHasHess>> {
+    static constexpr bool value = true;
+};
+template <class M, class = void>
+struct HasWideEval {
+    static constexpr bool value = false;
+};
+template <class M>
+struct HasWideEval<M, std::enable_if_t<M::kWideEval>> {
     static constexpr bool value = true;
 };
 template <class M, class = void>
diff --git a/mahi-mpc_amd/csrc/sqp_group.h b/mahi-mpc_amd/csrc/sqp_group.h
--- a/mahi-mpc_amd/csrc/sqp_group.h
+++ b/mahi-mpc_amd/csrc/sqp_group.h
@@ -175,6 +175,54 @@
     }
 }
 
+template <class Model, int W, int LM, bool JAC, int SQ, int FD, int FU>
+__device__ __forceinline__ void group_model_w(bool lin, const double* lFq, const double* lFqd, const double* lFu,
+                                              const double* lxd, const double* lxs, const double* lus,
+                                              const double (*x)[Model::NX], const double (*u)[Model::NU],
+                                              double (*xd)[Model::NX], double (*Fq)[SQ], double (*Fqd)[FD],
+                                              double (*Fu)[FU]) {
+    constexpr int NX = Model::NX, NQ = Model::NQ, NU = Model::NU, NA = NX - NQ;
+    if constexpr (W == 1 || LM != 0) {
+#pragma unroll
+        for (int e = 0; e < W; ++e)
+            group_model<Model>(W == 1 ? lin : true, lFq, lFqd, lFu, lxd, lxs, lus, x[e], u[e], xd[e], JAC ? Fq[e] : nullptr,
+                               JAC ? Fqd[e] : nullptr, JAC ? Fu[e] : nullptr, JAC);
+    } else {
+        using T = dpack<W>;
+        T xw[NX], uw[NU], xdw[NX];
+#pragma unroll
+        for (int e = 0; e < W; ++e) {
+#pragma unroll
+            for (int i = 0; i < NX; ++i) xw[i].v[e] = x[e][i];
+#pragma unroll
+            for (int i = 0; i < NU; ++i) uw[i].v[e] = u[e][i];
+        }
+        if constexpr (JAC) {
+            T fq[SQ], fqd[FD], fu[FU];
+            Model::eval_acc_jac(xw, uw, xdw + NQ, fq, fqd, fu);
+#pragma unroll
+            for (int e = 0; e < W; ++e) {
+#pragma unroll
+                for (int i = 0; i < NQ; ++i) xd[e][i] = x[e][NQ + i];
+#pragma unroll
+                for (int i = 0; i < NA; ++i) xd[e][NQ + i] = xdw[NQ + i].v[e];
+#pragma unroll
+                for (int i = 0; i < NA * NQ; ++i) Fq[e][i] = fq[i].v[e];
+#pragma unroll
+                for (int i = 0; i < FD; ++i) Fqd[e][i] = fqd[i].v[e];
+#pragma unroll
+                for (int i = 0; i < FU; ++i) Fu[e][i] = fu[i].v[e];
+            }
+        } else {
+            Model::eval(xw, uw, xdw);
+#pragma unroll
+            for (int e = 0; e < W; ++e)
+#pragma unroll
+                for (int i = 0; i < NX; ++i) xd[e][i] = xdw[i].v[e];
+        }
+    }
+}
+
 template <class Model, bool BOUNDED = false, bool XB = false, bool EXACT = false>
 __global__ __launch_bounds__(64) void sqp_group_kernel(SolveParams p, GroupWork gw) {
     constexpr bool MEHR = false;
@@ -243,6 +291,9 @@
     [[maybe_unused]] double* const sVr = sCu + N * NY;
     const double* const trg = p.traj + ii * (int64_t)N * NX;
 
+    constexpr bool PAIR = HasWideEval<Model>::value && !BOUNDED && !XB;
+    constexpr int WD = PAIR ? 2 : 1;
+    constexpr int WA = WD, WJ = WD, WW = WD;
     const double* w = p.weights + ii * p.w_stride;
     double Q[NX], R[NU], Rm[NU], up[NU];
 #pragma unroll
@@ -255,6 +306,40 @@
     }
     double lbv[NU], ubv[NU];
     load_bounds<NU, BOUNDED, IB>(p, inst, lbv, ubv);
+    [[maybe_unused]] double px0[NX], pxv[WD][NX], puv[WD][NU], prv[WD][NX];
+    [[maybe_unused]] auto pro_k = [&](int k0, int e) { return k0 + e * G <= N ? k0 + e * G : (k0 <= N ? k0 : N); };
+    [[maybe_unused]] auto pro_load = [&](int k0, double (*xv)[NX], double (*uv)[NU], double (*rv)[NX]) {
+        const double* Vin = p.V + ii * (int64_t)NV;
+#pragma unroll
+        for (int e = 0; e < WD; ++e) {
+            const int k = pro_k(k0, e), ku = k < N ? k : N - 1;
+#pragma unroll
+            for (int r = 0; r < NX; ++r) rv[e][r] = trg[ku * NX + r];
+        }
+        if (p.init_zero) {
+#pragma unroll
+            for (int e = 0; e < WD; ++e) {
+#pragma unroll
+                for (int r = 0; r < NX; ++r) xv[e][r] = 0.0;
+#pragma unroll
+                for (int c = 0; c < NU; ++c) uv[e][c] = 0.0;
+            }
+        } else {
+#pragma unroll
+            for (int e = 0; e < WD; ++e) {
+                const int k = pro_k(k0, e), ku = k < N ? k : N - 1;
+#pragma unroll
+                for (int r = 0; r < NX; ++r) xv[e][r] = Vin[k * ND + r];
+#pragma unroll
+                for (int c = 0; c < NU; ++c) uv[e][c] = Vin[ku * ND + NX + c];
+            }
+        }
+    };
+    if constexpr (PAIR) {
+#pragma unroll
+        for (int r = 0; r < NX; ++r) px0[r] = p.x0[ii * NX + r];
+        pro_load(gl, pxv, puv, prv);
+    }
     constexpr bool DIST = (NS < G);
     static_assert(!MEHR || DIST, "Mehrotra's rule: lane-distributed path");
     constexpr bool CAFF = IsControlAffine<Model>::value;
@@ -325,7 +410,22 @@
     if constexpr (LOPS) {
         for (int i = gl; i < KC; i += G) sKc[i] = (i == NX - 1) ? h : 0.0;
     }
-    {
+    if constexpr (PAIR) {
+        const bool hold = p.init_hold != 0;
+        for (int k0 = gl; k0 <= N; k0 += WD * G) {
+            if (k0 != gl) pro_load(k0, pxv, puv, prv);
+#pragma unroll
+            for (int e = 0; e < WD; ++e) {
+                const int k = pro_k(k0, e), ku = k < N ? k : N - 1;
+#pragma unroll
+                for (int r = 0; r < NX; ++r) sX[k * NX + r] = (k == 0 || hold) ? px0[r] : pxv[e][r];
+#pragma unroll
+                for (int c = 0; c < NU; ++c) sU[ku * NU + c] = puv[e][c];
+#pragma unroll
+                for (int r = 0; r < NX; ++r) sR[ku * NX + r] = prv[e][r];
+            }
+        }
+    } else {
         const double* Vin = p.V + ii * (int64_t)NV;
         for (int k = gl; k <= N; k += G) {
 #pragma unroll
@@ -397,6 +497,11 @@
     double kkt = 0.0, mu = resume ? p.tail_mu[slot] : 0.0, pg_prev = (BOUNDED && resume) ? p.tail_mub[slot] : INFINITY;
     bool done = !valid;
     constexpr bool FUSE_FWD = true;
+    auto with_lin = [&](auto wd_c, auto&& body) {
+        if constexpr (decltype(wd_c)::value == 1) body(std::integral_constant<int, -1>{});
+        else if (p.is_linear != 0) body(std::integral_constant<int, 1>{});
+        else body(std::integral_constant<int, 0>{});
+    };
     bool fwd_ready = false;
     double J0n = 0.0, c1n = 0.0, cmaxn = 0.0;
     int nfn = 0;
@@ -412,38 +517,63 @@
             c1 = 0.0;
             cmax = 0.0;
             nonfinite = 0;
-            for (int k = gl; k < N; k += G) {
-                double x[NX], u[NU], xd[NX], Fq[SQ], Fqd[FD], Fu[FU];
-#pragma unroll
-                for (int r = 0; r < NX; ++r) x[r] = sX[k * NX + r];
-#pragma unroll
-                for (int c = 0; c < NU; ++c) u[c] = sU[k * NU + c];
-                group_model<Model>(lin, lFq, lFqd, lFu, lxd, lxs, up, x, u, xd, Fq, Fqd, Fu, true);
-#pragma unroll
-                for (int i = 0; i < FQ; ++i) sFq[k * FQ + i] = h * Fq[i];
-#pragma unroll
-                for (int i = 0; i < FD; ++i) sFqd[k * FD + i] = h * Fqd[i];
-#pragma unroll
-                for (int i = 0; i < FU; ++i) sFu[k * FU + i] = h * Fu[i];
-#pragma unroll
-                for (int r = 0; r < NX; ++r) {
-                    const double F = fma(h, xd[r], x[r]);
-                    sF[k * NX + r] = F;
-                    const double c = F - sX[(k + 1) * NX + r];
-                    sC[k * NX + r] = c;
-                    cmax = fmax(cmax, fabs(c));
-                    c1 += fabs(c);
-                    nonfinite |= !isfinite(c);
-                    const double e = F - tr[k * NX + r];
-                    J0 = fma(e * Q[r], e, J0);
-                }
-#pragma unroll
-                for (int c = 0; c < NU; ++c) {
-                    const double um = (k == 0) ? up[c] : sU[(k - 1) * NU + c];
-                    const double dif = u[c] - um;
-                    J0 = fma(dif * R[c], dif, fma(u[c] * Rm[c], u[c], J0));
-                }
-            }
+            with_lin(std::integral_constant<int, WA>{}, [&](auto lm_c) {
+                constexpr int LM = decltype(lm_c)::value;
+                for (int k0 = gl; k0 < N; k0 += WA * G) {
+                    int kk[WA];
+                    double x[WA][NX], u[WA][NU], xd[WA][NX], Fq[WA][SQ], Fqd[WA][FD], Fu[WA][FU];
+#pragma unroll
+                    for (int e = 0; e < WA; ++e) {
+                        kk[e] = (e == 0 || k0 + e * G < N) ? k0 + e * G : k0;
+#pragma unroll
+                        for (int r = 0; r < NX; ++r) x[e][r] = sX[kk[e] * NX + r];
+#pragma unroll
+                        for (int c = 0; c < NU; ++c) u[e][c] = sU[kk[e] * NU + c];
+                    }
+                    group_model_w<Model, WA, LM, true, SQ, FD, FU>(lin, lFq, lFqd, lFu, lxd, lxs, up, x, u, xd, Fq, Fqd, Fu);
+                    double cd[WA][NX], er[WA][NX];
+#pragma unroll
+                    for (int e = 0; e < WA; ++e) {
+                        const int k = kk[e];
+#pragma unroll
+                        for (int i = 0; i < FQ; ++i) sFq[k * FQ + i] = h * Fq[e][i];
+#pragma unroll
+                        for (int i = 0; i < FD; ++i) sFqd[k * FD + i] = h * Fqd[e][i];
+#pragma unroll
+                        for (int i = 0; i < FU; ++i) sFu[k * FU + i] = h * Fu[e][i];
+#pragma unroll
+                        for (int r = 0; r < NX; ++r) {
+                            const double F = fma(h, xd[e][r], x[e][r]);
+                            sF[k * NX + r] = F;
+                            cd[e][r] = F - sX[(k + 1) * NX + r];
+                            sC[k * NX + r] = cd[e][r];
+                            er[e][r] = F - tr[k * NX + r];
+                        }
+                    }
+#pragma unroll
+                    for (int e = 0; e < WA; ++e) {
+                        const int k = kk[e];
+                        double Js = J0, cs = c1;
+#pragma unroll
+                        for (int r = 0; r < NX; ++r) {
+                            const double c = cd[e][r];
+                            cmax = fmax(cmax, fabs(c));
+                            cs += fabs(c);
+                            nonfinite |= !isfinite(c);
+                            Js = fma(er[e][r] * Q[r], er[e][r], Js);
+                        }
+#pragma unroll
+                        for (int c = 0; c < NU; ++c) {
+                            const double um = (k == 0) ? up[c] : sU[(k - 1) * NU + c];
+                            const double dif = u[e][c] - um;
+                            Js = fma(dif * R[c], dif, fma(u[e][c] * Rm[c], u[e][c], Js));
+                        }
+                        const bool on = e == 0 || k0 + e * G < N;
+                        J0 = on ? Js : J0;
+                        c1 = on ? cs : c1;
+                    }
+                }
+            });
         }
         double lsum = 0.0, cmpl0 = 0.0, cmplmu = 0.0;
         if constexpr (XB) {
@@ -1578,45 +1708,78 @@
         MMPC_PHASE(9);
         if constexpr (EXACT) {
             __builtin_amdgcn_wave_barrier();
-            auto w_stage = [&](int k) {
-                double x[NX], u[NU], la[NA], W[KZ * KZ];
-#pragma unroll
-                for (int r2 = 0; r2 < NX; ++r2) x[r2] = sX[k * NX + r2];
-#pragma unroll
-                for (int c = 0; c < NU; ++c) u[c] = sU[k * NU + c];
-#pragma unroll
-                for (int s2 = 0; s2 < NA; ++s2) la[s2] = h * sD[(k + 1) * NX + NQ + s2];
+            auto w_stages = [&](const int (&kk)[WW]) {
+                double x[WW][NX], u[WW][NU], la[WW][NA], W[WW][KZ * KZ];
+#pragma unroll
+                for (int e = 0; e < WW; ++e) {
+                    const int k = kk[e];
+#pragma unroll
+                    for (int r2 = 0; r2 < NX; ++r2) x[e][r2] = sX[k * NX + r2];
+#pragma unroll
+                    for (int c = 0; c < NU; ++c) u[e][c] = sU[k * NU + c];
+#pragma unroll
+                    for (int s2 = 0; s2 < NA; ++s2) la[e][s2] = h * sD[(k + 1) * NX + NQ + s2];
+                }
                 if constexpr (WLDS) __builtin_amdgcn_wave_barrier();
-                Model::eval_hess(x, u, la, W);
-                if constexpr (WLDS) {
-                    static_assert(!WLDS || PK >= NX, "write order of the W pass");
-#pragma unroll
-                    for (int r2 = 0; r2 < NX; ++r2)
-#pragma unroll
-                        for (int j = r2; j < KZ; ++j)
-                            if (WPack<Model>::idx(r2, j) >= 0) sW[k * PK + WPack<Model>::idx(r2, j)] = W[r2 * KZ + j];
+                if constexpr (WW == 1) {
+                    Model::eval_hess(x[0], u[0], la[0], W[0]);
                 } else {
-                    double* const dst = wH + k * HW;
-#pragma unroll
-                    for (int r2 = 0; r2 < NX; ++r2)
-#pragma unroll
-                        for (int j = 0; j < KZ; ++j)
-                            if (!w_struct_zero<Model>(r2, j) || !w_zeros_stored) dst[r2 * KZ + j] = W[r2 * KZ + j];
-                    if constexpr (!CAFF) {
-#pragma unroll
-                        for (int a = 0; a < NU; ++a)
-#pragma unroll
-                            for (int b = 0; b < NU; ++b) dst[NX * KZ + a * NU + b] = W[(NX + a) * KZ + NX + b];
-                    }
-                }
+                    using T = dpack<WW>;
+                    T xw[NX], uw[NU], lw[NA], Ww[KZ * KZ];
+#pragma unroll
+                    for (int e = 0; e < WW; ++e) {
+#pragma unroll
+                        for (int i = 0; i < NX; ++i) xw[i].v[e] = x[e][i];
+#pragma unroll
+                        for (int i = 0; i < NU; ++i) uw[i].v[e] = u[e][i];
+#pragma unroll
+                        for (int i = 0; i < NA; ++i) lw[i].v[e] = la[e][i];
+                    }
+                    Model::eval_hess(xw, uw, lw, Ww);
+#pragma unroll
+                    for (int e = 0; e < WW; ++e)
+#pragma unroll
+                        for (int i = 0; i < KZ * KZ; ++i) W[e][i] = Ww[i].v[e];
+                }
+#pragma unroll
+                for (int e = 0; e < WW; ++e) {
+                    const int k = kk[e];
+                    if constexpr (WLDS) {
+                        static_assert(!WLDS || PK >= NX, "write order of the W pass");
+#pragma unroll
+                        for (int r2 = 0; r2 < NX; ++r2)
+#pragma unroll
+                            for (int j = r2; j < KZ; ++j)
+                                if (WPack<Model>::idx(r2, j) >= 0) sW[k * PK + WPack<Model>::idx(r2, j)] = W[e][r2 * KZ + j];
+                    } else {
+                        double* const dst = wH + k * HW;
+#pragma unroll
+                        for (int r2 = 0; r2 < NX; ++r2)
+#pragma unroll
+                            for (int j = 0; j < KZ; ++j)
+                                if (!w_struct_zero<Model>(r2, j) || !w_zeros_stored) dst[r2 * KZ + j] = W[e][r2 * KZ + j];
+                        if constexpr (!CAFF) {
+#pragma unroll
+                            for (int a = 0; a < NU; ++a)
+#pragma unroll
+                                for (int b = 0; b < NU; ++b) dst[NX * KZ + a * NU + b] = W[e][(NX + a) * KZ + NX + b];
+                        }
+                    }
+                }
+            };
+            auto w_pair = [&](int k0) {
+                int kk[WW];
+#pragma unroll
+                for (int e = 0; e < WW; ++e) kk[e] = (e == 0 || k0 + e * G < N) ? k0 + e * G : k0;
+                w_stages(kk);
             };
             if constexpr (WLDS) {
-                for (int k0 = ((N - 1) / G) * G; k0 >= 0; k0 -= G)
-                    if (k0 + gl < N) w_stage(k0 + gl);
+                for (int k0 = ((N - 1) / (WW * G)) * (WW * G); k0 >= 0; k0 -= WW * G)
+                    if (k0 + gl < N) w_pair(k0 + gl);
                 MMPC_PHASE(9);
                 __builtin_amdgcn_wave_barrier();
             } else {
-                for (int k = gl; k < N; k += G) w_stage(k);
+                for (int k = gl; k < N; k += WW * G) w_pair(k);
                 w_zeros_stored = true;
                 MMPC_PHASE(9);
                 __builtin_amdgcn_fence(__ATOMIC_RELEASE, "workgroup");
@@ -1899,15 +2062,33 @@
             }
             __builtin_amdgcn_wave_barrier();
             double dj = 0.0;
-            for (int k = gl; k < N; k += G) {
-#pragma unroll
-                for (int q = 0; q < NX; ++q) dj = fma(2.0 * Q[q] * (sF[k * NX + q] - tr[k * NX + q]), sD[(k + 1) * NX + q], dj);
-#pragma unroll
-                for (int c = 0; c < NU; ++c) {
-                    const double uk = sU[k * NU + c], duk = sDU[k * NU + c];
-                    const double um = (k == 0) ? up[c] : sU[(k - 1) * NU + c];
-                    const double dum = (k == 0) ? 0.0 : sDU[(k - 1) * NU + c];
-                    dj = fma(2.0 * R[c] * (uk - um), duk - dum, fma(2.0 * Rm[c] * uk, duk, dj));
+            for (int k0 = gl; k0 < N; k0 += WD * G) {
+                double ef[WD][NX], ad[WD][NX], uk[WD][NU], duk[WD][NU], um[WD][NU], dum[WD][NU];
+#pragma unroll
+                for (int e = 0; e < WD; ++e) {
+                    const int k = (e == 0 || k0 + e * G < N) ? k0 + e * G : k0;
+#pragma unroll
+                    for (int q = 0; q < NX; ++q) {
+                        ef[e][q] = sF[k * NX + q] - tr[k * NX + q];
+                        ad[e][q] = sD[(k + 1) * NX + q];
+                    }
+#pragma unroll
+                    for (int c = 0; c < NU; ++c) {
+                        uk[e][c] = sU[k * NU + c];
+                        duk[e][c] = sDU[k * NU + c];
+                        um[e][c] = (k == 0) ? up[c] : sU[(k - 1) * NU + c];
+                        dum[e][c] = (k == 0) ? 0.0 : sDU[(k - 1) * NU + c];
+                    }
+                }
+#pragma unroll
+                for (int e = 0; e < WD; ++e) {
+                    double ds = dj;
+#pragma unroll
+                    for (int q = 0; q < NX; ++q) ds = fma(2.0 * Q[q] * ef[e][q], ad[e][q], ds);
+#pragma unroll
+                    for (int c = 0; c < NU; ++c)
+                        ds = fma(2.0 * R[c] * (uk[e][c] - um[e][c]), duk[e][c] - dum[e][c], fma(2.0 * Rm[c] * uk[e][c], duk[e][c], ds));
+                    dj = (e == 0 || k0 + e * G < N) ? ds : dj;
                 }
             }
             dJ = group_sum(dj);
@@ -1960,61 +2141,88 @@
         int nft = 0;
         auto trial = [&](auto jac_c, double& Jt, double& ct, double& lt) {
             constexpr bool JAC = decltype(jac_c)::value;
-            for (int k = gl; k < N; k += G) {
-                double x[NX], u[NU], xd[NX];
-#pragma unroll
-                for (int r = 0; r < NX; ++r) x[r] = fma(alpha, sDX[k * NX + r], sX[k * NX + r]);
-#pragma unroll
-                for (int c = 0; c < NU; ++c) {
-                    u[c] = fma(alpha, sDU[k * NU + c], sU[k * NU + c]);
-                    if (BOUNDED) u[c] = proj(u[c], lbv[c], ubv[c]);
-                }
-                if constexpr (JAC) {
-                    double Fq[SQ], Fqd[FD], Fu[FU];
-                    group_model<Model>(lin, lFq, lFqd, lFu, lxd, lxs, up, x, u, xd, Fq, Fqd, Fu, true);
-#pragma unroll
-                    for (int i = 0; i < FQ; ++i) sFq[k * FQ + i] = h * Fq[i];
-#pragma unroll
-                    for (int i = 0; i < FD; ++i) sFqd[k * FD + i] = h * Fqd[i];
-#pragma unroll
-                    for (int i = 0; i < FU; ++i) sFu[k * FU + i] = h * Fu[i];
-#pragma unroll
-                    for (int r = 0; r < NX; ++r) {
-                        const double F = fma(h, xd[r], x[r]);
-                        sF[k * NX + r] = F;
-                        const double c = F - fma(alpha, sDX[(k + 1) * NX + r], sX[(k + 1) * NX + r]);
-                        sC[k * NX + r] = c;
-                        ctm = fmax(ctm, fabs(c));
-                        ct += fabs(c);
-                        nft |= !isfinite(c);
-                        const double er = F - tr[k * NX + r];
-                        Jt = fma(er * Q[r], er, Jt);
-                    }
-                } else {
-                    group_model<Model>(lin, lFq, lFqd, lFu, lxd, lxs, up, x, u, xd, nullptr, nullptr, nullptr, false);
-#pragma unroll
-                    for (int r = 0; r < NX; ++r) {
-                        const double F = fma(h, xd[r], x[r]);
-                        const double er = F - tr[k * NX + r];
-                        Jt = fma(er * Q[r], er, Jt);
-                        ct += fabs(F - fma(alpha, sDX[(k + 1) * NX + r], sX[(k + 1) * NX + r]));
-                    }
-                }
-#pragma unroll
-                for (int c = 0; c < NU; ++c) {
-                    double um = (k == 0) ? up[c] : fma(alpha, sDU[(k - 1) * NU + c], sU[(k - 1) * NU + c]);
-                    if (BOUNDED && k > 0) um = proj(um, lbv[c], ubv[c]);
-                    const double dif = u[c] - um;
-                    Jt = fma(dif * R[c], dif, fma(u[c] * Rm[c], u[c], Jt));
-                }
-                if constexpr (XB) {
-#pragma unroll
-                    for (int j = 0; j < NY; ++j) {
-                        const double y = j < NX ? fma(alpha, sDX[(k + 1) * NX + j], sX[(k + 1) * NX + j]) : u[j - NX];
-                        lt += ip_log_slacks(y, yl[j], yu[j]);
-                    }
-                }
-            }
+            constexpr int WT = JAC ? WJ : 1;
+            with_lin(std::integral_constant<int, WT>{}, [&](auto lm_c) {
+                constexpr int LM = decltype(lm_c)::value;
+                for (int k0 = gl; k0 < N; k0 += WT * G) {
+                    int kk[WT];
+                    double x[WT][NX], u[WT][NU], xd[WT][NX];
+                    [[maybe_unused]] double Fq[WT][SQ], Fqd[WT][FD], Fu[WT][FU];
+#pragma unroll
+                    for (int e = 0; e < WT; ++e) {
+                        const int k = kk[e] = (e == 0 || k0 + e * G < N) ? k0 + e * G : k0;
+#pragma unroll
+                        for (int r = 0; r < NX; ++r) x[e][r] = fma(alpha, sDX[k * NX + r], sX[k * NX + r]);
+#pragma unroll
+                        for (int c = 0; c < NU; ++c) {
+                            u[e][c] = fma(alpha, sDU[k * NU + c], sU[k * NU + c]);
+                            if (BOUNDED) u[e][c] = proj(u[e][c], lbv[c], ubv[c]);
+                        }
+                    }
+                    group_model_w<Model, WT, LM, JAC, SQ, FD, FU>(lin, lFq, lFqd, lFu, lxd, lxs, up, x, u, xd, Fq, Fqd, Fu);
+                    double cd[WT][NX], er[WT][NX];
+#pragma unroll
+                    for (int e = 0; e < WT; ++e) {
+                        const int k = kk[e];
+                        if constexpr (JAC) {
+#pragma unroll
+                            for (int i = 0; i < FQ; ++i) sFq[k * FQ + i] = h * Fq[e][i];
+#pragma unroll
+                            for (int i = 0; i < FD; ++i) sFqd[k * FD + i] = h * Fqd[e][i];
+#pragma unroll
+                            for (int i = 0; i < FU; ++i) sFu[k * FU + i] = h * Fu[e][i];
+                        }
+#pragma unroll
+                        for (int r = 0; r < NX; ++r) {
+                            const double F = fma(h, xd[e][r], x[e][r]);
+                            if constexpr (JAC) sF[k * NX + r] = F;
+                            if constexpr (JAC) {
+                                cd[e][r] = F - fma(alpha, sDX[(k + 1) * NX + r], sX[(k + 1) * NX + r]);
+                                sC[k * NX + r] = cd[e][r];
+                                er[e][r] = F - tr[k * NX + r];
+                            } else {
+                                er[e][r] = F - tr[k * NX + r];
+                                cd[e][r] = F - fma(alpha, sDX[(k + 1) * NX + r], sX[(k + 1) * NX + r]);
+                            }
+                        }
+                    }
+#pragma unroll
+                    for (int e = 0; e < WT; ++e) {
+                        const int k = kk[e];
+                        double Js = Jt, cs = ct, ls = lt;
+#pragma unroll
+                        for (int r = 0; r < NX; ++r) {
+                            if constexpr (JAC) {
+                                ctm = fmax(ctm, fabs(cd[e][r]));
+                                cs += fabs(cd[e][r]);
+                                nft |= !isfinite(cd[e][r]);
+                                Js = fma(er[e][r] * Q[r], er[e][r], Js);
+                            } else {
+                                Js = fma(er[e][r] * Q[r], er[e][r], Js);
+                                cs += fabs(cd[e][r]);
+                            }
+                        }
+#pragma unroll
+                        for (int c = 0; c < NU; ++c) {
+                            double um = (k == 0) ? up[c] : fma(alpha, sDU[(k - 1) * NU + c], sU[(k - 1) * NU + c]);
+                            if (BOUNDED && k > 0) um = proj(um, lbv[c], ubv[c]);
+                            const double dif = u[e][c] - um;
+                            Js = fma(dif * R[c], dif, fma(u[e][c] * Rm[c], u[e][c], Js));
+                        }
+                        if constexpr (XB) {
+#pragma unroll
+                            for (int j = 0; j < NY; ++j) {
+                                const double y = j < NX ? fma(alpha, sDX[(k + 1) * NX + j], sX[(k + 1) * NX + j]) : u[e][j - NX];
+                                ls += ip_log_slacks(y, yl[j], yu[j]);
+                            }
+                        }
+                        const bool on = e == 0 || k0 + e * G < N;
+                        Jt = on ? Js : Jt;
+                        ct = on ? cs : ct;
+                        lt = on ? ls : lt;
+                    }
+                }
+            });
         };
         bool jac_trial = false;
         for (int ls = 0; ls < 30; ++ls) {
@@ -2071,16 +2279,44 @@
             }
             if constexpr (!MEHR) mub = mub_next;
         } else {
-            for (int k = gl; k <= N; k += G) {
-                if (k > 0) {
-#pragma unroll
-                    for (int r = 0; r < NX; ++r) sX[k * NX + r] = fma(alpha, sDX[k * NX + r], sX[k * NX + r]);
-                }
-                if (k < N) {
-#pragma unroll
-                    for (int c = 0; c < NU; ++c) {
-                        const double un = fma(alpha, sDU[k * NU + c], sU[k * NU + c]);
-                        sU[k * NU + c] = BOUNDED ? proj(un, lbv[c], ubv[c]) : un;
+            for (int k0 = gl; k0 <= N; k0 += WD * G) {
+                int kk[WD], ku[WD];
+                double xn[WD][NX], un[WD][NU];
+#pragma unroll
+                for (int e = 0; e < WD; ++e) {
+                    const int k = kk[e] = (e == 0 || k0 + e * G <= N) ? k0 + e * G : k0;
+                    if constexpr (WD == 1) {
+                        ku[e] = k;
+                        if (k > 0) {
+#pragma unroll
+                            for (int r = 0; r < NX; ++r) xn[e][r] = fma(alpha, sDX[k * NX + r], sX[k * NX + r]);
+                        }
+                        if (k < N) {
+#pragma unroll
+                            for (int c = 0; c < NU; ++c) un[e][c] = fma(alpha, sDU[k * NU + c], sU[k * NU + c]);
+                        }
+                    } else {
+                        ku[e] = k < N ? k : N - 1;
+#pragma unroll
+                        for (int r = 0; r < NX; ++r) {
+                            const double xo = sX[k * NX + r];
+                            xn[e][r] = k > 0 ? fma(alpha, sDX[k * NX + r], xo) : xo;
+                        }
+#pragma unroll
+                        for (int c = 0; c < NU; ++c) un[e][c] = fma(alpha, sDU[ku[e] * NU + c], sU[ku[e] * NU + c]);
+                    }
+                }
+                if constexpr (WD > 1) __builtin_amdgcn_wave_barrier();
+#pragma unroll
+                for (int e = 0; e < WD; ++e) {
+                    const int k = kk[e];
+                    if (WD > 1 || k > 0) {
+#pragma unroll
+                        for (int r = 0; r < NX; ++r) sX[k * NX + r] = xn[e][r];
+                    }
+                    if (k < N) {
+#pragma unroll
+                        for (int c = 0; c < NU; ++c) sU[ku[e] * NU + c] = BOUNDED ? proj(un[e][c], lbv[c], ubv[c]) : un[e][c];
                     }
                 }
             }
diff --git a/mahi-mpc_amd/csrc/two_link_fast.h b/mahi-mpc_amd/csrc/two_link_fast.h
--- a/mahi-mpc_amd/csrc/two_link_fast.h
+++ b/mahi-mpc_amd/csrc/two_link_fast.h
@@ -1,46 +1,100 @@
 #pragma once
+#include <type_traits>
+
 #include "fast_trig.h"
 
 namespace mmpc {
 
+template <int W>
+struct dpack {
+    static constexpr int width = W;
+    double v[W];
+    dpack() = default;
+    MMPC_HD dpack(double s) {
+        for (int e = 0; e < W; ++e) v[e] = s;
+    }
+#define MMPC_DPACK_OP(NAME, EXPR)                              \
+    MMPC_HD friend dpack NAME(const dpack& a, const dpack& b) { \
+        dpack r;                                               \
+        for (int e = 0; e < W; ++e) r.v[e] = EXPR;             \
+        return r;                                              \
+    }
+    MMPC_DPACK_OP(operator+, a.v[e] + b.v[e])
+    MMPC_DPACK_OP(operator-, a.v[e] - b.v[e])
+    MMPC_DPACK_OP(operator*, a.v[e] * b.v[e])
+    MMPC_DPACK_OP(operator/, a.v[e] / b.v[e])
+#undef MMPC_DPACK_OP
+    MMPC_HD friend dpack operator-(const dpack& a) {
+        dpack r;
+        for (int e = 0; e < W; ++e) r.v[e] = -a.v[e];
+        return r;
+    }
+    MMPC_HD friend dpack fma(const dpack& a, const dpack& b, const dpack& c) {
+        dpack r;
+        for (int e = 0; e < W; ++e) r.v[e] = __builtin_fma(a.v[e], b.v[e], c.v[e]);
+        return r;
+    }
+};
+
 struct TwoLinkFast {
     static constexpr double kG = 9.81;
-    struct Terms {
-        double sA, cA, sB, cB, sAB, cAB, E, F, iD, nA, nB;
+    template <class T>
+    struct TermsT {
+        T sA, cA, sB, cB, sAB, cAB, E, F, iD, nA, nB;
     };
-    MMPC_HD static void terms(const double* x, const double* u, Terms& t) {
+    using Terms = TermsT<double>;
+    template <class T>
+    MMPC_HD static void terms(const T* x, const T* u, TermsT<T>& t) {
         const trig_cptr TK = trig_table();
-        sincos_fast(TK, x[0], &t.sA, &t.cA);
-        sincos_fast(TK, x[1], &t.sB, &t.cB);
+        if constexpr (std::is_same<T, double>::value) {
+            sincos_fast(TK, x[0], &t.sA, &t.cA);
+            sincos_fast(TK, x[1], &t.sB, &t.cB);
+        } else {
+            constexpr int W = T::width;
+            double a[2 * W], s[2 * W], c[2 * W];
+            for (int e = 0; e < W; ++e) {
+                a[e] = x[0].v[e];
+                a[W + e] = x[1].v[e];
+            }
+            sincos_fast_w<2 * W>(TK, a, s, c);
+            for (int e = 0; e < W; ++e) {
+                t.sA.v[e] = s[e];
+                t.cA.v[e] = c[e];
+                t.sB.v[e] = s[W + e];
+                t.cB.v[e] = c[W + e];
+            }
+        }
         t.cAB = fma(t.cA, t.cB, -t.sA * t.sB);
         t.sAB = fma(t.sA, t.cB, t.cA * t.sB);
         t.E = 1.0 + t.cB;
         t.F = fma(2.0, t.cB, 3.0);
         t.iD = 1.0 / fma(t.cB, t.cB, -2.0);
-        const double dA = x[2], dB = x[3], TA = u[0], TB = u[1], dS = dA + dB;
+        const T dA = x[2], dB = x[3], TA = u[0], TB = u[1], dS = dA + dB;
         t.nA = fma(-t.E, TB, TA) + t.sB * fma(dS, dS, t.cB * dA * dA) + kG * fma(t.cB, t.cAB, -2.0 * t.cA);
         t.nB = fma(t.E, TA, -t.F * TB) + t.sB * fma(t.F * dA, dA, t.E * dB * fma(2.0, dA, dB)) +
                kG * fma(2.0 + t.cB, t.cAB, -2.0 * t.E * t.cA);
     }
-    MMPC_HD static void eval(const double* x, const double* u, double* xd) {
-        Terms t;
+    template <class T>
+    MMPC_HD static void eval(const T* x, const T* u, T* xd) {
+        TermsT<T> t;
         terms(x, u, t);
         xd[0] = x[2];
         xd[1] = x[3];
         xd[2] = -t.nA * t.iD;
         xd[3] = t.nB * t.iD;
     }
-    MMPC_HD static void grads(const double* x, const double* u, const Terms& t, double* gA, double* gB) {
-        const double dA = x[2], dB = x[3], TA = u[0], TB = u[1], dS = dA + dB;
-        const double c2s2 = fma(t.cB, t.cB, -t.sB * t.sB);
+    template <class T>
+    MMPC_HD static void grads(const T* x, const T* u, const TermsT<T>& t, T* gA, T* gB) {
+        const T dA = x[2], dB = x[3], TA = u[0], TB = u[1], dS = dA + dB;
+        const T c2s2 = fma(t.cB, t.cB, -t.sB * t.sB);
         gA[0] = kG * fma(-t.cB, t.sAB, 2.0 * t.sA);
         gA[1] = t.sB * TB + t.cB * dS * dS + c2s2 * dA * dA - kG * fma(t.sB, t.cAB, t.cB * t.sAB);
         gA[2] = 2.0 * t.sB * fma(t.cB, dA, dS);
         gA[3] = 2.0 * t.sB * dS;
         gA[4] = 1.0;
         gA[5] = -t.E;
-        const double Q = fma(t.F * dA, dA, t.E * dB * fma(2.0, dA, dB));
-        const double P = dA * fma(2.0, dA, 2.0 * dB) + dB * dB;
+        const T Q = fma(t.F * dA, dA, t.E * dB * fma(2.0, dA, dB));
+        const T P = dA * fma(2.0, dA, 2.0 * dB) + dB * dB;
         gB[0] = kG * fma(-(2.0 + t.cB), t.sAB, 2.0 * t.E * t.sA);
         gB[1] = fma(-t.sB, TA, 2.0 * t.sB * TB) + fma(t.cB, Q, -t.sB * t.sB * P) +
                 kG * (fma(-t.sB, t.cAB, -(2.0 + t.cB) * t.sAB) + 2.0 * t.sB * t.cA);
@@ -49,15 +103,16 @@
         gB[4] = t.E;
         gB[5] = -t.F;
     }
-    MMPC_HD static void eval_acc_jac(const double* x, const double* u, double* acc, double* Fq, double* Fqd, double* Fu) {
-        Terms t;
+    template <class T>
+    MMPC_HD static void eval_acc_jac(const T* x, const T* u, T* acc, T* Fq, T* Fqd, T* Fu) {
+        TermsT<T> t;
         terms(x, u, t);
-        double gA[6], gB[6];
+        T gA[6], gB[6];
         grads(x, u, t, gA, gB);
-        const double aA = -t.nA * t.iD, aB = t.nB * t.iD;
+        const T aA = -t.nA * t.iD, aB = t.nB * t.iD;
         acc[0] = aA;
         acc[1] = aB;
-        const double rD = -2.0 * t.cB * t.sB * t.iD;
+        const T rD = -2.0 * t.cB * t.sB * t.iD;
         Fq[0] = -gA[0] * t.iD;
         Fq[1] = fma(-gA[1], t.iD, -aA * rD);
         Fq[2] = gB[0] * t.iD;
@@ -71,30 +126,31 @@
         Fu[2] = gB[4] * t.iD;
         Fu[3] = gB[5] * t.iD;
     }
-    MMPC_HD static void eval_hess(const double* x, const double* u, const double* lam, double* W) {
-        Terms t;
+    template <class T>
+    MMPC_HD static void eval_hess(const T* x, const T* u, const T* lam, T* W) {
+        TermsT<T> t;
         terms(x, u, t);
-        double gA[6], gB[6];
+        T gA[6], gB[6];
         grads(x, u, t, gA, gB);
-        const double dA = x[2], dB = x[3], TA = u[0], TB = u[1], dS = dA + dB;
-        const double l0 = -lam[0], l1 = lam[1];
-        const double c2s2 = fma(t.cB, t.cB, -t.sB * t.sB);
-        const double Q = fma(t.F * dA, dA, t.E * dB * fma(2.0, dA, dB));
-        const double P = dA * fma(2.0, dA, 2.0 * dB) + dB * dB;
-        const double A00 = kG * fma(-t.cB, t.cAB, 2.0 * t.cA);
-        const double A01 = kG * fma(t.sB, t.sAB, -t.cB * t.cAB);
-        const double A11 = t.cB * TB - t.sB * dS * dS - 4.0 * t.cB * t.sB * dA * dA -
+        const T dA = x[2], dB = x[3], TA = u[0], TB = u[1], dS = dA + dB;
+        const T l0 = -lam[0], l1 = lam[1];
+        const T c2s2 = fma(t.cB, t.cB, -t.sB * t.sB);
+        const T Q = fma(t.F * dA, dA, t.E * dB * fma(2.0, dA, dB));
+        const T P = dA * fma(2.0, dA, 2.0 * dB) + dB * dB;
+        const T A00 = kG * fma(-t.cB, t.cAB, 2.0 * t.cA);
+        const T A01 = kG * fma(t.sB, t.sAB, -t.cB * t.cAB);
+        const T A11 = t.cB * TB - t.sB * dS * dS - 4.0 * t.cB * t.sB * dA * dA -
                            2.0 * kG * fma(t.cB, t.cAB, -t.sB * t.sAB);
-        const double A12 = 2.0 * fma(t.cB, dS, c2s2 * dA), A13 = 2.0 * t.cB * dS, A15 = t.sB;
-        const double A22 = 2.0 * t.sB * t.E, A23 = 2.0 * t.sB, A33 = 2.0 * t.sB;
-        const double B00 = kG * fma(-(2.0 + t.cB), t.cAB, 2.0 * t.E * t.cA);
-        const double B01 = kG * (fma(t.sB, t.sAB, -(2.0 + t.cB) * t.cAB) - 2.0 * t.sB * t.sA);
-        const double B11 = fma(-t.cB, TA, 2.0 * t.cB * TB) - t.sB * fma(3.0 * t.cB, P, Q) +
+        const T A12 = 2.0 * fma(t.cB, dS, c2s2 * dA), A13 = 2.0 * t.cB * dS, A15 = t.sB;
+        const T A22 = 2.0 * t.sB * t.E, A23 = 2.0 * t.sB, A33 = 2.0 * t.sB;
+        const T B00 = kG * fma(-(2.0 + t.cB), t.cAB, 2.0 * t.E * t.cA);
+        const T B01 = kG * (fma(t.sB, t.sAB, -(2.0 + t.cB) * t.cAB) - 2.0 * t.sB * t.sA);
+        const T B11 = fma(-t.cB, TA, 2.0 * t.cB * TB) - t.sB * fma(3.0 * t.cB, P, Q) +
                            2.0 * kG * (fma(-t.E, t.cAB, t.sB * t.sAB) + t.cB * t.cA);
-        const double B12 = fma(t.cB, 2.0 * fma(t.F, dA, t.E * dB), -t.sB * t.sB * (4.0 * dA + 2.0 * dB));
-        const double B13 = 2.0 * dS * fma(t.E, t.cB, -t.sB * t.sB), B14 = -t.sB, B15 = 2.0 * t.sB;
-        const double B22 = 2.0 * t.F * t.sB, B23 = 2.0 * t.E * t.sB, B33 = 2.0 * t.E * t.sB;
-        double H[6][6];
+        const T B12 = fma(t.cB, 2.0 * fma(t.F, dA, t.E * dB), -t.sB * t.sB * (4.0 * dA + 2.0 * dB));
+        const T B13 = 2.0 * dS * fma(t.E, t.cB, -t.sB * t.sB), B14 = -t.sB, B15 = 2.0 * t.sB;
+        const T B22 = 2.0 * t.F * t.sB, B23 = 2.0 * t.E * t.sB, B33 = 2.0 * t.E * t.sB;
+        T H[6][6];
 #pragma unroll
         for (int i = 0; i < 6; ++i)
 #pragma unroll
@@ -109,17 +165,17 @@
         H[2][2] = fma(l0, A22, l1 * B22);
         H[2][3] = fma(l0, A23, l1 * B23);
         H[3][3] = fma(l0, A33, l1 * B33);
-        double gp[6];
+        T gp[6];
 #pragma unroll
         for (int j = 0; j < 6; ++j) gp[j] = fma(l0, gA[j], l1 * gB[j]);
-        const double psi = fma(l0, t.nA, l1 * t.nB);
-        const double Dp = -2.0 * t.cB * t.sB, Dpp = -2.0 * c2s2;
-        const double iD = t.iD, iD2 = iD * iD;
+        const T psi = fma(l0, t.nA, l1 * t.nB);
+        const T Dp = -2.0 * t.cB * t.sB, Dpp = -2.0 * c2s2;
+        const T iD = t.iD, iD2 = iD * iD;
 #pragma unroll
         for (int i = 0; i < 6; ++i)
 #pragma unroll
             for (int j = i; j < 6; ++j) {
-                double v = H[i][j] * iD;
+                T v = H[i][j] * iD;
                 if (j == 1) v = fma(-gp[i] * Dp, iD2, v);
                 if (i == 1) v = fma(-gp[j] * Dp, iD2, v);
                 if (i == 1 && j == 1) v = fma(psi, fma(2.0 * Dp * Dp, iD, -Dpp) * iD2, v);
```
